# BolinLai/CSTS

Measured on AMD Instinct MI355X. Metric: clips/sec training (fwd+bwd) CSTS-Ego4D 16x256^2 bf16, higher is better.
Workload: dtype bf16; 1 GPU; CSTS_Ego4D_Gaze_Forecast.yaml train step (fwd + KLDiv + 0.05*EgoNCE + bwd + clip + AdamW), 16x256^2 video + 24 kHz STFT audio, b=4/GPU; mode=train, global_batch=4, frames=16, crop=256, parallelism=dp1, step=hip_graph, hip_graph=True, rccl_ranks=1

## Files before the change

csts_amd/csrc/attention.hip:

```cpp
#include <type_traits>
#include <utility>
#include "common.h"

#ifndef CSTS_ATTN_PART
#define CSTS_ATTN_PART 0
#endif
#ifndef CSTS_DKV_DEPTH
#define CSTS_DKV_DEPTH 4
#endif
#ifndef CSTS_DKV_SWZ
#define CSTS_DKV_SWZ 0
#endif

#ifdef CSTS_ATTN_STAMPS
#if CSTS_ATTN_PART == 1
__device__ unsigned long long g_attn_stamps[4096];
#else
static __device__ unsigned long long g_attn_stamps[4096];
#endif
#define AT_STAMP() do { if (stamp_on && nstamp < 4000) g_attn_stamps[nstamp++] = (unsigned long long)__builtin_amdgcn_s_memtime(); } while (0)
#if CSTS_ATTN_PART == 1
extern "C" int csts_debug_attn_stamps(unsigned long long* dst_host) {
  return (int)hipMemcpyFromSymbol(dst_host, HIP_SYMBOL(g_attn_stamps), sizeof(unsigned long long) * 4096);
}
// ... 1430 lines not shown
  CSTS_REQUIRE(strides_ok((a)->q_strides, (a)->dtype) && strides_ok((a)->k_strides, (a)->dtype) &&      \
                   strides_ok((a)->v_strides, (a)->dtype),                                             \
               "strides must keep 16-byte row alignment");                                              \
  if ((a)->mask_mode == CSTS_MASK_SPATIAL)                                                              \
  CSTS_REQUIRE((a)->mask_HW > 0 && (a)->Nq < (1 << 20) && (a)->Nq == (a)->mask_T * (a)->mask_HW + (a)->mask_T && (a)->Nk == (a)->Nq, "spatial mask needs Nq == Nk == T*HW + T < 2^20")

template <int HD, bool F32>
static bool launch_fwd(const AttnRoute& r, const AttnP& p, dim3 grid, hipStream_t stream) {
  const size_t sm = smem_fwd<HD, F32>();
  if (r.fwd == FWD_FAST) hipLaunchKernelGGL(attn_fwd_fast_kernel, grid, dim3(256), sm, stream, p);
  else hipLaunchKernelGGL((attn_fwd_kernel<HD, F32>), grid, dim3(256), sm, stream, p);
  return true;
}
template <int HD, bool F32>
static bool launch_dq(const AttnRoute& r, const AttnP& p, dim3 grid, hipStream_t stream) {
  const size_t sm = smem_bwd<HD, F32>();
  if (r.dq == DQ_FAST128) {
    constexpr size_t sm4 = (size_t)2 * 128 * 2 * Cfg<96, false>::LD_ROW * 2;
    if (!csts_dyn_lds_optin(reinterpret_cast<const void*>(&attn_dq_fast_kernel<4>), (int)sm4)) return false;
    hipLaunchKernelGGL(attn_dq_fast_kernel<4>, grid, dim3(256), sm4, stream, p);
  } else if (r.dq == DQ_FAST64) hipLaunchKernelGGL(attn_dq_fast_kernel<2>, grid, dim3(256), sm, stream, p);
  else hipLaunchKernelGGL((attn_dq_kernel<HD, F32>), grid, dim3(256), sm, stream, p);
  return true;
}
template <int HD, bool F32>
static bool launch_dkv(const AttnRoute& r, const AttnP& p, dim3 grid, hipStream_t stream) {
  const size_t sm = smem_bwd<HD, F32>() + (size_t)Cfg<HD, F32>::KVBLK * 4 * sizeof(float);
  if (r.dkv == DKV_FAST) return csts_attn_dkv_fast_launch(p, grid, stream);
  if constexpr (HD == 192 && !F32) {
    if (r.dkv == DKV_PLAIN) {
      hipLaunchKernelGGL((attn_dkv_kernel<192, false, false>), grid, dim3(256), sm, stream, p);
      return true;
    }
  }
  hipLaunchKernelGGL((attn_dkv_kernel<HD, F32, true>), grid, dim3(256), sm, stream, p);
  return true;
}
#define LAUNCH_BY_TYPE(fn, a, ...)                                                                                   \
  ((a)->head_dim == 96 ? ((a)->dtype == CSTS_F32 ? fn<96, true>(__VA_ARGS__) : fn<96, false>(__VA_ARGS__))           \
                       : ((a)->dtype == CSTS_F32 ? fn<192, true>(__VA_ARGS__) : fn<192, false>(__VA_ARGS__)))

static void launch_reduce(const csts_attn_args* a, const AttnP& p, hipStream_t stream) {
  const int64_t total = (int64_t)2 * a->B * a->H * a->Nk * a->head_dim / 8;
  hipLaunchKernelGGL(attn_dkv_reduce_kernel, dim3((unsigned)std::min<int64_t>(cdiv(total, 256), 4096)), dim3(256), 0, stream, p,
                     a->head_dim);
}

extern "C" int csts_attn_fwd(const csts_attn_args* a, hipStream_t stream) {
  ATTN_COMMON_CHECKS(a);
  CSTS_REQUIRE(a->O && a->LSE && aligned16(a->O) && strides_ok(a->o_strides, a->dtype), "bad output");
  AttnP p; fill(a, p);
  AttnRoute r;
  CSTS_REQUIRE(attn_route(a, &r), "no route");
  dim3 grid((unsigned)cdiv(a->Nq, 128), a->H, a->B);
  CSTS_REQUIRE(LAUNCH_BY_TYPE(launch_fwd, a, r, p, grid, stream), "hipFuncSetAttribute(MaxDynamicSharedMemorySize) failed on this device");
  CSTS_LAUNCH_CHECK();
  return 0;
}

extern "C" size_t csts_attn_bwd_workspace(const csts_attn_args* a) {
  AttnRoute r;
  return attn_route(a, &r) ? r.ws_bytes : 0;
}

extern "C" int csts_attn_route(const csts_attn_args* a, char* buf, int buflen, int* nsplit, int* q_chunk) {
  CSTS_REQUIRE(buf != nullptr && buflen > 0 && nsplit != nullptr && q_chunk != nullptr, "null pointer");
  AttnRoute r;
  CSTS_REQUIRE(attn_route(a, &r), "no route: null args, empty problem, or head_dim not 96 / 192");
  *nsplit = r.nsplit;
  *q_chunk = r.q_chunk;
  const int hd = a->head_dim;
  const char* t = a->dtype == CSTS_BF16 ? "false" : "true";
  char fwd[48] = "attn_fwd_fast_kernel", dq[48] = "", dkv[48] = "attn_bwd_fused_kernel";
  if (r.fwd == FWD_GENERIC) snprintf(fwd, sizeof fwd, "attn_fwd_kernel<%d,%s>", hd, t);
  if (r.dq == DQ_GENERIC) snprintf(dq, sizeof dq, "attn_dq_kernel<%d,%s>", hd, t);
  else if (r.dq != DQ_NONE) snprintf(dq, sizeof dq, "attn_dq_fast_kernel<%d>", r.dq == DQ_FAST128 ? 4 : 2);
  if (r.dkv == DKV_SLOW) snprintf(dkv, sizeof dkv, "attn_dkv_kernel<%d,%s,true>", hd, t);
  else if (r.dkv != DKV_ONE_PASS) snprintf(dkv, sizeof dkv, "attn_dkv_kernel<%d,false,false>", hd);
  const int n = snprintf(buf, buflen, "%s;%s;%s;%s", fwd, dq, dkv, r.nsplit > 1 ? "attn_dkv_reduce_kernel" : "");
  CSTS_REQUIRE(n < buflen, "buffer too small");
  return 0;
}

extern "C" int csts_attn_bwd(const csts_attn_args* a, void* workspace, size_t ws_bytes, hipStream_t stream) {
  ATTN_COMMON_CHECKS(a);
  CSTS_REQUIRE(a->O && a->LSE && a->dO && a->delta && a->dQ && a->dK && a->dV, "null backward operand");
  CSTS_REQUIRE(aligned16(a->dO) && aligned16(a->dQ) && aligned16(a->dK) && aligned16(a->dV), "alignment");
  CSTS_REQUIRE(strides_ok(a->do_strides, a->dtype) && strides_ok(a->dq_strides, a->dtype) &&
                   strides_ok(a->dk_strides, a->dtype) && strides_ok(a->dv_strides, a->dtype) &&
                   strides_ok(a->o_strides, a->dtype), "strides must keep 16-byte row alignment");
  AttnP p; fill(a, p);
  AttnRoute r;
  CSTS_REQUIRE(attn_route(a, &r), "no route");
  p.nsplit = r.nsplit; p.q_chunk = r.q_chunk;
  if (r.nsplit > 1) {
    if (workspace == nullptr || ws_bytes < r.ws_bytes) CSTS_FAIL("workspace too small [workspace != nullptr && ws_bytes >= csts_attn_bwd_workspace(a)]");
    p.ws = reinterpret_cast<float*>(workspace);
  }
  if (r.dkv == DKV_ONE_PASS) {
    hipLaunchKernelGGL((attn_bwd_fused_kernel<96>), dim3((unsigned)p.nsplit, (unsigned)(a->B * a->H)), dim3(256), 0, stream, p);
  } else {
    dim3 grid_dq((unsigned)cdiv(a->Nq, 128), a->H, a->B);
    CSTS_REQUIRE(LAUNCH_BY_TYPE(launch_dq, a, r, p, grid_dq, stream), "hipFuncSetAttribute(MaxDynamicSharedMemorySize) failed on this device");
    CSTS_LAUNCH_CHECK();
    dim3 grid_dkv((unsigned)cdiv(a->Nk, 128), p.nsplit, a->B * a->H);
    CSTS_REQUIRE(LAUNCH_BY_TYPE(launch_dkv, a, r, p, grid_dkv, stream), "hipFuncSetAttribute(MaxDynamicSharedMemorySize) failed on this device");
  }
  CSTS_LAUNCH_CHECK();
  if (r.nsplit > 1) {
    launch_reduce(a, p, stream);
    CSTS_LAUNCH_CHECK();
  }
  return 0;
}

extern "C" int csts_attn_probs(const csts_attn_args* a, float* probs, hipStream_t stream) {
  ATTN_COMMON_CHECKS(a);
  CSTS_REQUIRE(a->LSE && probs, "null pointer");
  AttnP p; fill(a, p);
  const int64_t total = (int64_t)a->B * a->H * a->Nq * a->Nk;
  hipLaunchKernelGGL(attn_probs_kernel, dim3((unsigned)std::min<int64_t>(cdiv(total, 256), 4096)), dim3(256), 0, stream, p,
                     a->head_dim, probs);
  CSTS_LAUNCH_CHECK();
  return 0;
}
#else
}
bool csts_attn_dkv_fast_launch(const csts_attn::AttnP& p, dim3 grid, hipStream_t stream) {
  constexpr size_t smf = (size_t)2 * 128 * 2 * (CSTS_DKV_SWZ ? 128 : Cfg<96, false>::LD_ROW) * 2 + 2 * 2 * 128 * sizeof(float);
  if (!csts_dyn_lds_optin(reinterpret_cast<const void*>(&attn_dkv_kernel<96, false, false>), (int)smf)) return false;
  hipLaunchKernelGGL((attn_dkv_kernel<96, false, false>), grid, dim3(256), smf, stream, p);
  return true;
}
#endif
```

csts_amd/csrc/norm.hip:

```cpp
#include "common.h"

#include <utility>

namespace {

constexpr int MAXV = 12;
constexpr int LN_BWD_WAVES = 8;

template <bool F32> __device__ __forceinline__ float ldt(const void* p, int64_t i) {
  if constexpr (F32) return reinterpret_cast<const float*>(p)[i];
  else return h16_lo((unsigned)reinterpret_cast<const unsigned short*>(p)[i]);
}
template <bool F32> __device__ __forceinline__ void stt(void* p, int64_t i, float v) {
  if constexpr (F32) reinterpret_cast<float*>(p)[i] = v;
  else reinterpret_cast<bf16*>(p)[i] = (bf16)v;
}
template <bool F32> __device__ __forceinline__ void ld8t(const void* p, int64_t i, float (&o)[8]) {
  if constexpr (F32) {
    const float4* q = reinterpret_cast<const float4*>(reinterpret_cast<const float*>(p) + i);
    const float4 a = q[0], b = q[1];
    o[0] = a.x; o[1] = a.y; o[2] = a.z; o[3] = a.w; o[4] = b.x; o[5] = b.y; o[6] = b.z; o[7] = b.w;
  } else {
    const uint4 r = *reinterpret_cast<const uint4*>(reinterpret_cast<const bf16*>(p) + i);
    o[0] = h16_lo(r.x); o[1] = h16_hi(r.x);
    o[2] = h16_lo(r.y); o[3] = h16_hi(r.y);
    o[4] = h16_lo(r.z); o[5] = h16_hi(r.z);
    o[6] = h16_lo(r.w); o[7] = h16_hi(r.w);
  }
}
template <bool F32> __device__ __forceinline__ void st8t(void* p, int64_t i, const float (&o)[8]) {
  if constexpr (F32) {
    float4* q = reinterpret_cast<float4*>(reinterpret_cast<float*>(p) + i);
    q[0] = make_float4(o[0], o[1], o[2], o[3]);
    q[1] = make_float4(o[4], o[5], o[6], o[7]);
  } else {
    bf16x8 v;
#pragma unroll
    for (int j = 0; j < 8; ++j) v[j] = (bf16)o[j];
    *reinterpret_cast<bf16x8*>(reinterpret_cast<bf16*>(p) + i) = v;
  }
}
template <int W, bool F32> __device__ __forceinline__ void ldw(const void* p, int64_t i, float (&o)[W]) {
  if constexpr (W == 8) ld8t<F32>(p, i, o);
  else o[0] = ldt<F32>(p, i);
}
template <int W, bool F32> __device__ __forceinline__ void stw(void* p, int64_t i, const float (&o)[W]) {
  if constexpr (W == 8) st8t<F32>(p, i, o);
  else stt<F32>(p, i, o[0]);
}
template <int GL> __device__ __forceinline__ float group_sum(float v) {
#pragma unroll
  for (int o = GL / 2; o > 0; o >>= 1) v += __shfl_xor(v, o, 64);
  return v;
}

__device__ __forceinline__ int64_t xcd_block(int64_t bid, int64_t nwg) {
#ifdef CSTS_LN_NO_XCD_MAP
  return bid;
#else
  const int64_t q = nwg >> 3, r = nwg & 7, xcd = bid & 7, slot = bid >> 3;
  return (xcd < r ? xcd * (q + 1) : r * (q + 1) + (xcd - r) * q) + slot;
#endif
}

template <int W, int GL, int NCH> struct Lane {
  int sub, C;
  int c0[W == 8 ? NCH : 1];
  bool act[W == 8 ? NCH : 1];
  __device__ __forceinline__ void form(int i) {
    if constexpr (W == 8) {
      const int c = (sub + GL * i) * 8;
      act[i] = c < C;
      c0[i] = min(c, C - 8);
    }
  }
  __device__ __forceinline__ bool on(int i) const {
    if constexpr (W == 8) return act[i];
    else return sub + GL * i < C;
  }
  __device__ __forceinline__ int st(int i) const {
    if constexpr (W == 8) return c0[i];
    else return sub + GL * i;
  }
  __device__ __forceinline__ int at(int i) const {
    if constexpr (W == 8) return c0[i];
    else return min(sub + GL * i, C - 1);
  }
  __device__ __forceinline__ void param(const float* p, int i, float (&o)[W]) const {
    if constexpr (W == 8) ld8t<true>(p, at(i), o);
    else o[0] = on(i) ? p[sub + GL * i] : 0.f;
  }
};

struct FwdAdd {
  const void* addend = nullptr;
  void* sum = nullptr;
};
template <int W, int GL, int NCH, int R, bool XF32, bool YF32>
__global__ __launch_bounds__(256) void ln_fwd_kernel(const void* __restrict__ x, const float* __restrict__ gamma,
                                                     const float* __restrict__ beta, void* __restrict__ y,
                                                     float* __restrict__ mean, float* __restrict__ rstd, int64_t rows,
                                                     int C, float eps, FwdAdd fa) {
  const int64_t bid = W == 8 ? xcd_block(blockIdx.x, gridDim.x) : (int64_t)blockIdx.x;
  const int64_t grp = (bid * 256 + threadIdx.x) / GL, ngrp = (int64_t)gridDim.x * 256 / GL;
  Lane<W, GL, NCH> ln{(int)(threadIdx.x % GL), C};
  float gm[NCH][W], bt[NCH][W];
#pragma unroll
  for (int i = 0; i < NCH; ++i) {
    ln.form(i);
    ln.param(gamma, i, gm[i]);
    ln.param(beta, i, bt[i]);
  }
  const float invC = 1.f / C;
  for (int64_t row0 = grp * R; row0 < rows; row0 += ngrp * R) {
    float v[R][NCH][W];
#pragma unroll
    for (int r = 0; r < R; ++r) {
      const int64_t row = min(row0 + r, rows - 1);
#pragma unroll
      for (int i = 0; i < NCH; ++i) {
        ldw<W, XF32>(x, row * C + ln.at(i), v[r][i]);
        if (fa.addend) {
          float a2[W];
          ldw<W, XF32>(fa.addend, row * C + ln.at(i), a2);
#pragma unroll
          for (int j = 0; j < W; ++j) {
            v[r][i][j] += a2[j];
            if constexpr (!XF32) v[r][i][j] = (float)(bf16)v[r][i][j];
          }
          if (ln.on(i) && row0 + r < rows) stw<W, XF32>(fa.sum, row * C + ln.st(i), v[r][i]);
        }
      }
    }
    constexpr int PH = W == 8 ? 1 : 3;
    float mu[R], rs[R];
#pragma unroll
    for (int ph = 0; ph < PH; ++ph)
#pragma unroll
      for (int r = 0; r < R; ++r) {
        if (PH == 1 || ph == 0) {
          float s = 0.f;
#pragma unroll
          for (int i = 0; i < NCH; ++i)
            if (ln.on(i)) {
#pragma unroll
              for (int j = 0; j < W; ++j) s += v[r][i][j];
            }
          mu[r] = group_sum<GL>(s) * invC;
        }
        if (PH == 1 || ph == 1) {
          float q = 0.f;
#pragma unroll
          for (int i = 0; i < NCH; ++i)
            if (ln.on(i)) {
#pragma unroll
              for (int j = 0; j < W; ++j) { const float d = v[r][i][j] - mu[r]; q += d * d; }
            }
          rs[r] = rsqrtf(group_sum<GL>(q) * invC + eps);
        }
        const int64_t row = row0 + r;
        if ((PH == 1 || ph == 2) && row < rows) {
#pragma unroll
          for (int i = 0; i < NCH; ++i)
            if (ln.on(i)) {
              float o[W];
#pragma unroll
              for (int j = 0; j < W; ++j) o[j] = (v[r][i][j] - mu[r]) * rs[r] * gm[i][j] + bt[i][j];
              stw<W, YF32>(y, row * C + ln.st(i), o);
            }
          if (ln.sub == 0) {
            if (mean) mean[row] = mu[r];
            if (rstd) rstd[row] = rs[r];
          }
        }
      }
  }
}

struct Copy16 {
  bf16* p = nullptr;
  const float* scale = nullptr;
  int64_t rps = 1;
  const void* dy2 = nullptr;
};
#ifndef CSTS_LN_BWD_R
#define CSTS_LN_BWD_R 1
#endif
#ifndef CSTS_LN_BWD_MINW
#define CSTS_LN_BWD_MINW 1
#endif
template <int W, int GL, int NCH, int R, bool DYF32, bool XF32>
__global__ __launch_bounds__(512, CSTS_LN_BWD_MINW) void ln_bwd_kernel(const void* __restrict__ dy, const void* __restrict__ x,
                                                         const float* __restrict__ gamma, const float* __restrict__ mean,
                                                         const float* __restrict__ rstd, void* __restrict__ dx,
                                                         const void* __restrict__ addend, float* __restrict__ ws, int64_t rows,
                                                         int C, const float* __restrict__ gamma1, Copy16 dx16) {
  extern __shared__ __attribute__((aligned(16))) float red[];
  const int64_t ro = (int64_t)blockIdx.y * rows;
  if (blockIdx.y == 1) gamma = gamma1;
  ws += (int64_t)blockIdx.y * gridDim.x * 2 * C;
  const int gib = threadIdx.x / GL;
  constexpr int GPB = 512 / GL;
  const int64_t bid = W == 8 ? xcd_block(blockIdx.x, gridDim.x) : (int64_t)blockIdx.x;
  const int64_t grp = bid * GPB + gib, ngrp = (int64_t)gridDim.x * GPB;
  Lane<W, GL, NCH> ln{(int)(threadIdx.x % GL), C};
  float gm[NCH][W], dg[NCH][W], db[NCH][W];
#pragma unroll
  for (int i = 0; i < NCH; ++i) {
    ln.form(i);
    ln.param(gamma, i, gm[i]);
#pragma unroll
    for (int j = 0; j < W; ++j) { dg[i][j] = 0.f; db[i][j] = 0.f; }
  }
  const float invC = 1.f / C;
  for (int64_t row0 = grp * R; row0 < rows; row0 += ngrp * R) {
    float d[R][NCH][W], xv[R][NCH][W], ad[R][NCH][W], mu[R], rs[R];
#pragma unroll
    for (int r = 0; r < R; ++r) {
      const int64_t row = ro + min(row0 + r, rows - 1);
      mu[r] = mean[row];
      rs[r] = rstd[row];
#pragma unroll
      for (int i = 0; i < NCH; ++i) {
        ldw<W, DYF32>(dy, row * C + ln.at(i), d[r][i]);
        if (dx16.dy2) {
          float d2[W];
          ldw<W, DYF32>(dx16.dy2, row * C + ln.at(i), d2);
#pragma unroll
          for (int j = 0; j < W; ++j) d[r][i][j] += d2[j];
        }
        ldw<W, XF32>(x, row * C + ln.at(i), xv[r][i]);
        if (addend) ldw<W, XF32>(addend, row * C + ln.at(i), ad[r][i]);
        else {
#pragma unroll
          for (int j = 0; j < W; ++j) ad[r][i][j] = 0.f;
        }
      }
    }
#pragma unroll
    for (int r = 0; r < R; ++r) {
      const bool live = row0 + r < rows;
      float s1 = 0.f, s2 = 0.f;
      float xh[NCH][W], g[NCH][W];
#pragma unroll
      for (int i = 0; i < NCH; ++i) {
        const bool ok = live && ln.on(i);
#pragma unroll
        for (int j = 0; j < W; ++j) {
          const float dd = ok ? d[r][i][j] : 0.f;
          xh[i][j] = ok ? (xv[r][i][j] - mu[r]) * rs[r] : 0.f;
          g[i][j] = dd * gm[i][j];
          dg[i][j] += dd * xh[i][j];
          db[i][j] += dd;
          s1 += g[i][j];
          s2 += g[i][j] * xh[i][j];
        }
      }
      s1 = group_sum<GL>(s1) * invC;
      s2 = group_sum<GL>(s2) * invC;
      if (live) {
        const int64_t row = ro + row0 + r;
#pragma unroll
        for (int i = 0; i < NCH; ++i)
          if (ln.on(i)) {
            float o[W];
#pragma unroll
            for (int j = 0; j < W; ++j) o[j] = rs[r] * (g[i][j] - s1 - xh[i][j] * s2) + ad[r][i][j];
            stw<W, XF32>(dx, row * C + ln.st(i), o);
            if (dx16.p) {
              if (dx16.scale) {
                const float sc = dx16.scale[(row0 + r) / dx16.rps];
#pragma unroll
                for (int j = 0; j < W; ++j) o[j] *= sc;
              }
              stw<W, false>(dx16.p, row * C + ln.st(i), o);
            }
          }
      }
    }
  }
#pragma unroll
  for (int i = 0; i < NCH; ++i)
    if (ln.on(i)) {
#pragma unroll
      for (int j = 0; j < W; ++j) {
        red[gib * 2 * C + ln.st(i) + j] = dg[i][j];
        red[gib * 2 * C + C + ln.st(i) + j] = db[i][j];
      }
    }
  __syncthreads();
  for (int i = threadIdx.x; i < 2 * C; i += blockDim.x) {
    float t = 0.f;
#pragma unroll(W == 8 ? 4 : GPB)
    for (int k = 0; k < GPB; ++k) t += red[k * 2 * C + i];
    ws[(int64_t)blockIdx.x * 2 * C + i] = t;
  }
}

template <int RL>
__global__ void reduce_rows_kernel(const float* __restrict__ ws, float* __restrict__ out, int64_t nrows, int64_t ncols,
                                   float scale) {
  __shared__ float red[RL][33];
  const int tx = threadIdx.x & 31, ty = threadIdx.x >> 5;
  const int64_t j = (int64_t)blockIdx.x * 32 + tx;
  float s = 0.f;
  if (j < ncols) {
    int64_t i = ty;
    for (; i + 3 * RL < nrows; i += 4 * RL) {
      const float a = ws[i * ncols + j], b = ws[(i + RL) * ncols + j], c = ws[(i + 2 * RL) * ncols + j],
                  d = ws[(i + 3 * RL) * ncols + j];
      s += a; s += b; s += c; s += d;
    }
    for (; i < nrows; i += RL) s += ws[i * ncols + j];
  }
  red[ty][tx] = s;
  __syncthreads();
  if (ty == 0 && j < ncols) {
    float t = 0.f;
#pragma unroll
    for (int r = 0; r < RL; ++r) t += red[r][tx];
    out[j] = t * scale;
  }
}

__global__ __launch_bounds__(1024) void reduce_rows_batched_kernel(const csts_reduce_desc* __restrict__ descs) {
  __shared__ float red[32][33];
  const csts_reduce_desc d = descs[blockIdx.y];
  const int tx = threadIdx.x & 31, ty = threadIdx.x >> 5;
  const int64_t j = (int64_t)blockIdx.x * 32 + tx;
  if ((int64_t)blockIdx.x * 32 >= d.ncols) return;
  float s = 0.f;
  if (j < d.ncols) {
    int64_t i = ty;
    for (; i + 3 * 32 < d.nrows; i += 4 * 32) {
      const float a = d.ws[i * d.ncols + j], b = d.ws[(i + 32) * d.ncols + j], c = d.ws[(i + 64) * d.ncols + j],
                  e = d.ws[(i + 96) * d.ncols + j];
      s += a; s += b; s += c; s += e;
    }
    for (; i < d.nrows; i += 32) s += d.ws[i * d.ncols + j];
  }
  red[ty][tx] = s;
  __syncthreads();
  if (ty == 0 && j < d.ncols) {
    float t = 0.f;
#pragma unroll
    for (int r = 0; r < 32; ++r) t += red[r][tx];
    d.out[j] = t * d.scale;
  }
}

__global__ __launch_bounds__(256) void reduce_rows_wide_kernel(const csts_reduce_desc* __restrict__ descs) {
  const csts_reduce_desc d = descs[blockIdx.y];
  const int64_t nvec = d.ncols >> 2;
  for (int64_t v = (int64_t)blockIdx.x * 256 + threadIdx.x; v < nvec; v += (int64_t)gridDim.x * 256) {
    float4 s = make_float4(0.f, 0.f, 0.f, 0.f);
    const float4* p = reinterpret_cast<const float4*>(d.ws) + v;
    int64_t i = 0;
    for (; i + 3 < d.nrows; i += 4) {
      const float4 a = p[i * nvec], b = p[(i + 1) * nvec], c = p[(i + 2) * nvec], e = p[(i + 3) * nvec];
      s.x += a.x; s.y += a.y; s.z += a.z; s.w += a.w;
      s.x += b.x; s.y += b.y; s.z += b.z; s.w += b.w;
      s.x += c.x; s.y += c.y; s.z += c.z; s.w += c.w;
      s.x += e.x; s.y += e.y; s.z += e.z; s.w += e.w;
    }
    for (; i < d.nrows; ++i) {
      const float4 a = p[i * nvec];
      s.x += a.x; s.y += a.y; s.z += a.z; s.w += a.w;
    }
    reinterpret_cast<float4*>(d.out)[v] = make_float4(s.x * d.scale, s.y * d.scale, s.z * d.scale, s.w * d.scale);
  }
}

}

extern "C" int csts_reduce_rows_wide(const csts_reduce_desc* device_descs, int n, int64_t max_ncols, hipStream_t stream) {
  CSTS_REQUIRE(device_descs != nullptr && n > 0 && n < 65536 && max_ncols > 0, "bad args");
  const unsigned gx = (unsigned)std::min<int64_t>(cdiv(max_ncols / 4, 256), 4096);
  hipLaunchKernelGGL(reduce_rows_wide_kernel, dim3(gx, (unsigned)n), dim3(256), 0, stream, device_descs);
  CSTS_LAUNCH_CHECK();
  return 0;
}

extern "C" int csts_reduce_rows_batched(const csts_reduce_desc* device_descs, int n, int64_t max_ncols, hipStream_t stream) {
  CSTS_REQUIRE(device_descs != nullptr && n > 0 && n < 65536 && max_ncols > 0, "bad args");
  hipLaunchKernelGGL(reduce_rows_batched_kernel, dim3((unsigned)cdiv(max_ncols, 32), (unsigned)n), dim3(1024), 0, stream,
                     device_descs);
  CSTS_LAUNCH_CHECK();
  return 0;
}

int csts_reduce_rows_launch(const float* ws, float* out, int64_t nrows, int64_t ncols, float scale, hipStream_t s) {
  const dim3 grid((unsigned)cdiv(ncols, 32));
  if (nrows > 64) hipLaunchKernelGGL(reduce_rows_kernel<32>, grid, dim3(1024), 0, s, ws, out, nrows, ncols, scale);
  else if (nrows > 8) hipLaunchKernelGGL(reduce_rows_kernel<8>, grid, dim3(256), 0, s, ws, out, nrows, ncols, scale);
  else hipLaunchKernelGGL(reduce_rows_kernel<2>, grid, dim3(64), 0, s, ws, out, nrows, ncols, scale);
  return 0;
}

extern "C" int csts_reduce_rows(const float* ws, float* out, int64_t nrows, int64_t ncols, float scale,
                                hipStream_t stream) {
  CSTS_REQUIRE(ws && out && nrows > 0 && ncols > 0, "bad args");
  csts_reduce_rows_launch(ws, out, nrows, ncols, scale, stream);
  CSTS_LAUNCH_CHECK();
  return 0;
}

#ifndef CSTS_LN_FWD_R
#define CSTS_LN_FWD_R 2
#endif
#ifndef CSTS_LN_BWD_CAP
#define CSTS_LN_BWD_CAP 512
#endif
struct LnForm { int W, GL, NCH, R; };
template <bool BWD> static constexpr LnForm LN_FORMS[8] = {
    {8, 16, 1, BWD ? CSTS_LN_BWD_R : CSTS_LN_FWD_R}, {8, 32, 1, BWD ? CSTS_LN_BWD_R : CSTS_LN_FWD_R},
    {8, 64, 1, BWD ? CSTS_LN_BWD_R : CSTS_LN_FWD_R}, {8, 64, 2, BWD ? 1 : 2},
    {1, 64, 2, 4}, {1, 64, 3, 4}, {1, 64, 6, 2}, {1, 64, 12, 1}};
static size_t ln_bwd_lds(const LnForm& f, int C) { return (size_t)(512 / f.GL) * 2 * C * sizeof(float); }
static int ln_form(bool bwd, int C, bool aligned) {
  const int vec = C <= 128 ? 0 : (C <= 256 ? 1 : (C <= 512 ? 2 : 3));
  if (aligned && C % 8 == 0 && !(bwd && ln_bwd_lds(LN_FORMS<true>[vec], C) > 65536)) return vec;
  return 4 + (C <= 128 ? 0 : (C <= 192 ? 1 : (C <= 384 ? 2 : 3)));
}
static bool all_aligned16(std::initializer_list<const void*> ptrs) {
  for (const void* q : ptrs)
    if (q != nullptr && !aligned16(q)) return false;
  return true;
}
static int64_t ln_bwd_blocks(int64_t rows, int C) {
  return std::min<int64_t>(cdiv(rows, LN_BWD_WAVES * LN_FORMS<true>[ln_form(true, C, false)].R), CSTS_LN_BWD_CAP);
}
template <class F, int... K> static void ln_pick(int k, F&& launch, std::integer_sequence<int, K...>) {
  ((k == K ? launch(std::integral_constant<int, K>{}) : void()), ...);
}

extern "C" int csts_layernorm_fwd(const void* x, int x_dt, const float* gamma, const float* beta, void* y, int y_dt,
                                  float* mean, float* rstd, int64_t rows, int C, float eps, hipStream_t stream) {
  return csts_layernorm_fwd_add(x, nullptr, nullptr, x_dt, gamma, beta, y, y_dt, mean, rstd, rows, C, eps, stream);
}

extern "C" int csts_layernorm_fwd_add(const void* x, const void* addend, void* sum_out, int x_dt, const float* gamma,
                                      const float* beta, void* y, int y_dt, float* mean, float* rstd, int64_t rows, int C,
                                      float eps, hipStream_t stream) {
  CSTS_REQUIRE(x && gamma && beta && y, "null pointer");
  CSTS_REQUIRE((addend == nullptr) == (sum_out == nullptr), "addend and sum_out: both or neither");
  CSTS_REQUIRE(rows > 0 && C > 0 && C <= 64 * MAXV, "C must be in (0, 768]");
  FwdAdd fa;
  fa.addend = addend; fa.sum = sum_out;
  const int form = ln_form(false, C, all_aligned16({x, y, gamma, beta, addend, sum_out}));
  const LnForm& f = LN_FORMS<false>[form];
  const dim3 grid((unsigned)std::min<int64_t>(cdiv(rows * f.GL, 256 * f.R), 4096));
  ln_pick(4 * form + 2 * (x_dt == CSTS_F32) + (y_dt == CSTS_F32), [&](auto k) {
    constexpr LnForm F = LN_FORMS<false>[decltype(k)::value / 4];
    hipLaunchKernelGGL((ln_fwd_kernel<F.W, F.GL, F.NCH, F.R, (decltype(k)::value & 2) != 0, (decltype(k)::value & 1) != 0>), grid,
                       dim3(256), 0, stream, x, gamma, beta, y, mean, rstd, rows, C, eps, fa);
  }, std::make_integer_sequence<int, 32>{});
  CSTS_LAUNCH_CHECK();
  return 0;
}

extern "C" size_t csts_layernorm_bwd_workspace(int64_t rows, int C) {
  return (size_t)ln_bwd_blocks(rows, C) * 2 * C * sizeof(float);
}

static void ln_bwd_launch(int segs, bool aligned, const void* dy, int dy_dt, const void* x, int x_dt, const float* const (&gamma)[2],
                          const float* mean, const float* rstd, void* dx, const void* addend, float* const (&dgb)[2], float* ws,
                          int64_t rows, int C, Copy16 c16, hipStream_t stream) {
  const int form = ln_form(true, C, aligned);
  const int64_t nb = ln_bwd_blocks(rows, C);
  const dim3 grid((unsigned)nb, (unsigned)segs);
  const size_t sh = ln_bwd_lds(LN_FORMS<true>[form], C);
  ln_pick(4 * form + 2 * (dy_dt == CSTS_F32) + (x_dt == CSTS_F32), [&](auto k) {
    constexpr LnForm F = LN_FORMS<true>[decltype(k)::value / 4];
    hipLaunchKernelGGL((ln_bwd_kernel<F.W, F.GL, F.NCH, F.R, (decltype(k)::value & 2) != 0, (decltype(k)::value & 1) != 0>), grid,
                       dim3(512), sh, stream, dy, x, gamma[0], mean, rstd, dx, addend, ws, rows, C, gamma[1], c16);
  }, std::make_integer_sequence<int, 32>{});
  for (int s = 0; s < segs && dgb[0] != nullptr; ++s) csts_reduce_rows_launch(ws + s * nb * 2 * C, dgb[s], nb, 2 * C, 1.f, stream);
}

extern "C" int csts_layernorm_bwd(const void* dy, int dy_dt, const void* x, int x_dt, const float* gamma,
                                  const float* mean, const float* rstd, void* dx, int dx_dt, const void* addend,
                                  void* dx_bf16, float* dgamma, float* dbeta, void* workspace, size_t ws_bytes,
                                  int64_t rows, int C, hipStream_t stream) {
  return csts_layernorm_bwd_ex(dy, nullptr, dy_dt, x, x_dt, gamma, mean, rstd, dx, dx_dt, addend, dx_bf16, nullptr, 1, dgamma,
                               dbeta, workspace, ws_bytes, rows, C, stream);
}

extern "C" int csts_layernorm_bwd_ex(const void* dy, const void* dy2, int dy_dt, const void* x, int x_dt, const float* gamma,
                                     const float* mean, const float* rstd, void* dx, int dx_dt, const void* addend,
                                     void* dx_bf16, const float* copy_row_scale, int64_t rows_per_scale,
                                     float* dgamma, float* dbeta, void* workspace, size_t ws_bytes, int64_t rows,
                                     int C, hipStream_t stream) {
  CSTS_REQUIRE(dy && x && gamma && mean && rstd && dx && workspace, "null pointer");
  CSTS_REQUIRE(copy_row_scale == nullptr || (dx_bf16 != nullptr && rows_per_scale > 0), "copy scale needs the bf16 copy and rows_per_scale > 0");
  Copy16 c16;
  c16.p = reinterpret_cast<bf16*>(dx_bf16); c16.scale = copy_row_scale; c16.rps = rows_per_scale > 0 ? rows_per_scale : 1;
  c16.dy2 = dy2;
  CSTS_REQUIRE(rows > 0 && C > 0 && C <= 64 * MAXV, "C must be in (0, 768]");
  CSTS_REQUIRE((dgamma == nullptr) == (dbeta == nullptr), "dgamma and dbeta: both or neither (neither = deferred second stage)");
  CSTS_REQUIRE(dgamma == nullptr || dbeta == dgamma + C, "dgamma/dbeta must be one contiguous [2*C] buffer");
  CSTS_REQUIRE(dx_dt == x_dt, "dx must have the dtype of x");
  const int64_t nb = ln_bwd_blocks(rows, C);
  CSTS_REQUIRE(ws_bytes >= (size_t)nb * 2 * C * sizeof(float), "workspace too small");
  ln_bwd_launch(1, all_aligned16({dy, dy2, x, dx, addend, dx_bf16, gamma}), dy, dy_dt, x, x_dt, {gamma, nullptr}, mean, rstd, dx,
                addend, {dgamma, nullptr}, reinterpret_cast<float*>(workspace), rows, C, c16, stream);
  CSTS_LAUNCH_CHECK();
  return 0;
}

extern "C" int csts_layernorm_bwd2(const void* dy, int dy_dt, const void* x, int x_dt, const float* gamma0,
                                   const float* gamma1, const float* mean, const float* rstd, void* dx, int dx_dt,
                                   float* dgb0, float* dgb1, void* workspace, size_t ws_bytes, int64_t rows, int C,
                                   hipStream_t stream) {
// ... 12 lines not shown
```

csts_amd/csrc/stencil.hip:

```cpp
#include "common.h"
#include <algorithm>
#include <cstdlib>
#include <cstring>
#include <initializer_list>
#include <vector>

namespace {

struct Geom {
  int B, C, HD;
  int Tf, Hf, Wf;
  int Tc, Hc, Wc;
  int st, sh, sw;
  int64_t f_bs, f_ts;
  int64_t c_bs, c_ts;
};

constexpr int VEC = 4;

__device__ __forceinline__ void ld4(const void* p, int dt, int64_t i, float (&o)[4]) {
  if (dt == CSTS_F32) {
    float4 a = *reinterpret_cast<const float4*>(reinterpret_cast<const float*>(p) + i);
    o[0] = a.x; o[1] = a.y; o[2] = a.z; o[3] = a.w;
  } else {
    bf16x4 a = *reinterpret_cast<const bf16x4*>(reinterpret_cast<const bf16*>(p) + i);
    o[0] = (float)a[0]; o[1] = (float)a[1]; o[2] = (float)a[2]; o[3] = (float)a[3];
  }
}
__device__ __forceinline__ void st4(void* p, int dt, int64_t i, const float (&o)[4]) {
  if (dt == CSTS_F32) {
    *reinterpret_cast<float4*>(reinterpret_cast<float*>(p) + i) = make_float4(o[0], o[1], o[2], o[3]);
  } else {
    bf16x4 a;
    a[0] = (bf16)o[0]; a[1] = (bf16)o[1]; a[2] = (bf16)o[2]; a[3] = (bf16)o[3];
    *reinterpret_cast<bf16x4*>(reinterpret_cast<bf16*>(p) + i) = a;
  }
}

struct FastDiv { unsigned m; int sh; int d; };
__device__ __forceinline__ int fdiv(int n, const FastDiv& f) { return (int)(((unsigned long long)(unsigned)n * f.m) >> f.sh); }
struct RowGeom {
  Geom g;
  int lt, lh, lw;
  FastDiv dNc, dHc, dWc;
  FastDiv dNf, dHf, dWf;
  FastDiv dN2, dH2, dW2;
  FastDiv dC4, dC8, dHD, dHeads;
};
__device__ __forceinline__ void decompf(int bt, const FastDiv& dN, const FastDiv& dH, const FastDiv& dW, int& b, int& t, int& h, int& w) {
  b = fdiv(bt, dN);
  int o = bt - b * dN.d;
  const int q = fdiv(o, dW);
  w = o - q * dW.d;
  t = fdiv(q, dH);
  h = q - t * dH.d;
}

__device__ __forceinline__ void decomp(int bt, int ntok, int H, int W, int& b, int& t, int& h, int& w) {
  b = bt / ntok;
  int o = bt - b * ntok;
  w = o % W; o /= W;
  h = o % H;
  t = o / H;
}

template <bool F32> __device__ __forceinline__ const void* bptr(const void* p, int64_t off) {
  if constexpr (F32) return reinterpret_cast<const float*>(p) + off;
  else return reinterpret_cast<const bf16*>(p) + off;
}
template <bool F32> __device__ __forceinline__ void* bptr(void* p, int64_t off) {
  if constexpr (F32) return reinterpret_cast<float*>(p) + off;
  else return reinterpret_cast<bf16*>(p) + off;
}

template <int V, bool F32> struct Raw { unsigned w[F32 ? V : V / 2]; };
template <int V, bool F32> __device__ __forceinline__ Raw<V, F32> raw_load(const void* base, int i) {
  Raw<V, F32> r;
  if constexpr (F32) {
    const uint4* q = reinterpret_cast<const uint4*>(reinterpret_cast<const float*>(base) + i);
#pragma unroll
    for (int k = 0; k < V / 4; ++k) { const uint4 a = q[k]; r.w[4 * k] = a.x; r.w[4 * k + 1] = a.y; r.w[4 * k + 2] = a.z; r.w[4 * k + 3] = a.w; }
  } else if constexpr (V == 8) {
    const uint4 a = *reinterpret_cast<const uint4*>(reinterpret_cast<const bf16*>(base) + i);
// ... 189 lines not shown
          float v[V];
          raw_cvt<V, F32>(raw[kh * 3 + kw], v);
          fmav<V>(acc, v, &wls[tap * (HD + WPAD)]);
        }
    };
    if constexpr (ALL27) {
      Raw<V, F32> r0[9], r1[9], r2[9];
      bool t0, t1, t2;
      slice_load(0, r0, t0); slice_load(1, r1, t1); slice_load(2, r2, t2);
      slice_mac(0, r0, t0); slice_mac(1, r1, t1); slice_mac(2, r2, t2);
    } else {
#pragma unroll 1
      for (int kt = 0; kt < 3; ++kt) {
        Raw<V, F32> raw[9];
        bool tvk;
        slice_load(kt, raw, tvk);
        slice_mac(kt, raw, tvk);
      }
    }
    if constexpr (!F32) {
#pragma unroll
      for (int j = 0; j < V; ++j) acc[j] = (float)(bf16)acc[j];
    }
    float s1 = 0.f;
    if (active) {
#pragma unroll
      for (int j = 0; j < V; ++j) s1 += acc[j];
    }
#pragma unroll
    for (int o = GL / 2; o > 0; o >>= 1) s1 += __shfl_xor(s1, o, 64);
    const float mu = s1 * invHD;
    float s2 = 0.f;
    if (active) {
#pragma unroll
      for (int j = 0; j < V; ++j) { const float d = acc[j] - mu; s2 += d * d; }
    }
#pragma unroll
    for (int o = GL / 2; o > 0; o >>= 1) s2 += __shfl_xor(s2, o, 64);
    const float rs = rsqrtf(s2 * invHD + eps);
    if (active) {
      const int64_t off = (int64_t)b * g.c_bs + (int64_t)(bt - b * ntok) * cts + c;
      raw_store<V, F32>(sl.conv[slot], off, acc);
      const float* gp = sl.gamma[slot] + cl;
      const float* bp = sl.beta[slot] + cl;
      float y[V];
#pragma unroll
      for (int q = 0; q < V / 4; ++q) {
        const float4 gq = *reinterpret_cast<const float4*>(gp + 4 * q), bq = *reinterpret_cast<const float4*>(bp + 4 * q);
        y[4 * q + 0] = (acc[4 * q + 0] - mu) * rs * gq.x + bq.x; y[4 * q + 1] = (acc[4 * q + 1] - mu) * rs * gq.y + bq.y;
        y[4 * q + 2] = (acc[4 * q + 2] - mu) * rs * gq.z + bq.z; y[4 * q + 3] = (acc[4 * q + 3] - mu) * rs * gq.w + bq.w;
      }
      raw_store<V, F32>(sl.y[slot], off, y);
      if (lane_in == 0) {
        const int64_t row = (int64_t)bt * H + head;
        sl.mean[slot][row] = mu;
        sl.rstd[slot][row] = rs;
      }
    }
  }
}

template <int N>
__device__ __forceinline__ void axis_cand(int f, int s, int ls, int nc, int (&k)[N], int (&o)[N], bool (&ok)[N]) {
#pragma unroll
  for (int i = 0; i < N; ++i) {
    int kk, n;
    if (N == 3) { kk = i; n = f + 1 - i; }
    else if (N == 2) { kk = ((f + 1) & 1) + 2 * i; n = f + 1 - kk; }
    else if (ls >= 0) { kk = (f + 1) & (s - 1); n = f + 1 - kk; }
    else { kk = (f + 1) % s; n = f + 1 - kk; }
    const int oo = ls >= 0 ? (n >> ls) : (n >= 0 ? n / s : -1);
    ok[i] = kk <= 2 && n >= 0 && oo < nc;
    k[i] = min(kk, 2);
    o[i] = min(max(oo, 0), nc - 1);
  }
}

struct Slots2 {
  const void* src[2];
  void* dst[2];
  const float* w[2];
};

template <int NT, int NH, int NW, bool CF32, bool FF32, int V>
__global__ __launch_bounds__(256, CSTS_DW_WAVES) void dwconv_transposed_kernel(RowGeom rg, Slots2 sl) {
  extern __shared__ __attribute__((aligned(16))) float wl[];
  const void* __restrict__ coarse = sl.src[blockIdx.y];
  const float* __restrict__ w = sl.w[blockIdx.y];
  void* __restrict__ fine = sl.dst[blockIdx.y];
  const Geom& g = rg.g;
  stage_weights_z(w, wl, g.HD);
  const int CQ = g.C / V;
  const int ntok = g.Tf * g.Hf * g.Wf;
  const int total = g.B * ntok * CQ;
  const int fts = (int)g.f_ts, cts = (int)g.c_ts;
  for (int idx = blockIdx.x * blockDim.x + threadIdx.x; idx < total; idx += gridDim.x * blockDim.x) {
    const int bt = fdiv(idx, V == 8 ? rg.dC8 : rg.dC4);
    const int c = (idx - bt * CQ) * V, cw = c - fdiv(c, rg.dHD) * g.HD;
    int b, ft, fh, fw;
    decompf(bt, rg.dNf, rg.dHf, rg.dWf, b, ft, fh, fw);
    int kt[NT], ot[NT], kh[NH], oh[NH], kw[NW], ow[NW];
    bool vt[NT], vh[NH], vw[NW];
    axis_cand<NT>(ft, g.st, rg.lt, g.Tc, kt, ot, vt);
    axis_cand<NH>(fh, g.sh, rg.lh, g.Hc, kh, oh, vh);
    axis_cand<NW>(fw, g.sw, rg.lw, g.Wc, kw, ow, vw);
#pragma unroll
    for (int i = 0; i < NT; ++i) ot[i] *= g.Hc * g.Wc * cts;
#pragma unroll
    for (int i = 0; i < NH; ++i) oh[i] *= g.Wc * cts;
#pragma unroll
    for (int i = 0; i < NW; ++i) ow[i] = ow[i] * cts + c;
    const void* cb = bptr<CF32>(coarse, (int64_t)b * g.c_bs);
    float acc[V];
#pragma unroll
    for (int j = 0; j < V; ++j) acc[j] = 0.f;
#pragma unroll
    for (int a = 0; a < NT; ++a) {
      Raw<V, CF32> raw[NH * NW];
#pragma unroll
      for (int e = 0; e < NH; ++e)
#pragma unroll
        for (int f = 0; f < NW; ++f) raw[e * NW + f] = raw_load<V, CF32>(cb, ot[a] + oh[e] + ow[f]);
#pragma unroll
      for (int e = 0; e < NH; ++e)
#pragma unroll
        for (int f = 0; f < NW; ++f) {
          const int tap = (vt[a] && vh[e] && vw[f]) ? kt[a] * 9 + kh[e] * 3 + kw[f] : 27;
          float v[V];
          raw_cvt<V, CF32>(raw[e * NW + f], v);
          fmav<V>(acc, v, &wl[tap * (g.HD + WPAD) + cw]);
        }
    }
    raw_store<V, FF32>(bptr<FF32>(fine, (int64_t)b * g.f_bs), (bt - b * ntok) * fts + c, acc);
  }
}

template <int NT>
__global__ __launch_bounds__(256, CSTS_DW_WAVES) void dwconv_transposed_s22_kernel(RowGeom rg, Slots2 sl) {
  extern __shared__ __attribute__((aligned(16))) float wl[];
  const bf16* __restrict__ coarse = reinterpret_cast<const bf16*>(sl.src[blockIdx.y]);
  bf16* __restrict__ fine = reinterpret_cast<bf16*>(sl.dst[blockIdx.y]);
  const Geom& g = rg.g;
  stage_weights_z(sl.w[blockIdx.y], wl, g.HD);
  const int CQ = g.C / 8;
  const int H2 = g.Hf >> 1, W2 = g.Wf >> 1;
  const int nblk = g.Tf * H2 * W2;
  const int total = g.B * nblk * CQ;
  const int fts = (int)g.f_ts, cts = (int)g.c_ts;
  for (int idx = blockIdx.x * blockDim.x + threadIdx.x; idx < total; idx += gridDim.x * blockDim.x) {
    const int bt = fdiv(idx, rg.dC8);
    const int c = (idx - bt * CQ) * 8, cw = c - fdiv(c, rg.dHD) * g.HD;
    int b, ft, mh, mw;
    decompf(bt, rg.dN2, rg.dH2, rg.dW2, b, ft, mh, mw);
    int kt[NT], ot[NT];
    bool vt[NT];
    axis_cand<NT>(ft, g.st, rg.lt, g.Tc, kt, ot, vt);
    const bool vh1 = mh + 1 < g.Hc, vw1 = mw + 1 < g.Wc;
    const int oh0 = mh * g.Wc * cts, oh1 = min(mh + 1, g.Hc - 1) * g.Wc * cts;
    const int ow0 = mw * cts + c, ow1 = min(mw + 1, g.Wc - 1) * cts + c;
    const bf16* cb = coarse + (int64_t)b * g.c_bs;
    float o00[8], o01[8], o10[8], o11[8];
#pragma unroll
    for (int j = 0; j < 8; ++j) { o00[j] = 0.f; o01[j] = 0.f; o10[j] = 0.f; o11[j] = 0.f; }
    Raw<8, false> raw[NT][4];
#pragma unroll
    for (int a = 0; a < NT; ++a) {
      const int tb = ot[a] * g.Hc * g.Wc * cts;
      raw[a][0] = raw_load<8, false>(cb, tb + oh0 + ow0);
      raw[a][1] = raw_load<8, false>(cb, tb + oh0 + ow1);
      raw[a][2] = raw_load<8, false>(cb, tb + oh1 + ow0);
      raw[a][3] = raw_load<8, false>(cb, tb + oh1 + ow1);
    }
#pragma unroll
    for (int a = 0; a < NT; ++a) {
      float i00[8], i01[8], i10[8], i11[8];
      raw_cvt<8, false>(raw[a][0], i00);
      raw_cvt<8, false>(raw[a][1], i01);
      raw_cvt<8, false>(raw[a][2], i10);
      raw_cvt<8, false>(raw[a][3], i11);
      const int t9 = kt[a] * 9;
      auto wrow = [&](bool ok, int kh, int kw) { return &wl[(ok ? t9 + kh * 3 + kw : 27) * (g.HD + WPAD) + cw]; };
      const bool v = vt[a];
      fmav<8>(o00, i00, wrow(v, 1, 1));
      fmav<8>(o01, i00, wrow(v, 1, 2));
      fmav<8>(o01, i01, wrow(v && vw1, 1, 0));
      fmav<8>(o10, i00, wrow(v, 2, 1));
      fmav<8>(o10, i10, wrow(v && vh1, 0, 1));
      fmav<8>(o11, i00, wrow(v, 2, 2));
      fmav<8>(o11, i01, wrow(v && vw1, 2, 0));
      fmav<8>(o11, i10, wrow(v && vh1, 0, 2));
      fmav<8>(o11, i11, wrow(v && vh1 && vw1, 0, 0));
    }
    bf16* fb = fine + (int64_t)b * g.f_bs;
    const int f00 = ((ft * g.Hf + 2 * mh) * g.Wf + 2 * mw) * fts + c;
    raw_store<8, false>(fb, f00, o00);
    raw_store<8, false>(fb, f00 + fts, o01);
    raw_store<8, false>(fb, f00 + g.Wf * fts, o10);
    raw_store<8, false>(fb, f00 + g.Wf * fts + fts, o11);
  }
}

struct WgSlots2 {
  const void* fine[2];
  const void* coarse[2];
  float* ws[2];
};
template <bool FF32, bool CF32>
__device__ __forceinline__ void dwconv_wgrad_body(const Geom& g, const void* __restrict__ fine, const void* __restrict__ coarse,
                                                  float* __restrict__ ws, int slab, int chunk, int bx, int by, int nbx, int tx, int ty,
                                                  int lanes, int nthr, float* __restrict__ red) {
  const int cl = 2 * tx;
  const int c = bx * slab + cl;
  const int ntok = g.Tc * g.Hc * g.Wc;
  const int total = g.B * ntok;
  const int beg = by * chunk, end = ty < lanes ? min(total, beg + chunk) : 0;
  const int fts = (int)g.f_ts, cts = (int)g.c_ts;
  float a0[27], a1[27];
#pragma unroll
  for (int k = 0; k < 27; ++k) { a0[k] = 0.f; a1[k] = 0.f; }
  int b = 0, ot = 0, oh = 0, ow = 0;
  if (beg + ty < end) decomp(beg + ty, ntok, g.Hc, g.Wc, b, ot, oh, ow);
  const int tstep = lanes;
  const char* fbase = reinterpret_cast<const char*>(fine);
  const char* cbase = reinterpret_cast<const char*>(coarse);
  constexpr unsigned FES = FF32 ? 4u : 2u, CES = CF32 ? 4u : 2u;
  for (int bt = beg + ty; bt < end; bt += tstep) {
    unsigned tof[3], hx[9];
    bool tv[3], hxv[9];
    {
      unsigned hof[3], xof[3];
      bool hv[3], xv[3];
#pragma unroll
      for (int k = 0; k < 3; ++k) {
        const int t = ot * g.st - 1 + k, h = oh * g.sh - 1 + k, x = ow * g.sw - 1 + k;
        tv[k] = (unsigned)t < (unsigned)g.Tf; tof[k] = (unsigned)(min(max(t, 0), g.Tf - 1) * g.Hf * g.Wf * fts);
        hv[k] = (unsigned)h < (unsigned)g.Hf; hof[k] = (unsigned)(min(max(h, 0), g.Hf - 1) * g.Wf * fts);
        xv[k] = (unsigned)x < (unsigned)g.Wf; xof[k] = (unsigned)(min(max(x, 0), g.Wf - 1) * fts + c);
      }
      const unsigned boff = (unsigned)((int)g.f_bs * b);
#pragma unroll
      for (int kh = 0; kh < 3; ++kh)
#pragma unroll
        for (int kw = 0; kw < 3; ++kw) { hx[kh * 3 + kw] = boff + hof[kh] + xof[kw]; hxv[kh * 3 + kw] = hv[kh] && xv[kw]; }
    }
    float c0, c1;
    {
      const unsigned coff = ((unsigned)((int)g.c_bs * b) + (unsigned)((bt - b * ntok) * cts + c)) * CES;
      if constexpr (CF32) {
        const float2 v = *reinterpret_cast<const float2*>(cbase + coff);
        c0 = v.x; c1 = v.y;
      } else {
        const unsigned v = *reinterpret_cast<const unsigned*>(cbase + coff);
        c0 = h16_lo(v); c1 = h16_hi(v);
      }
    }
    if constexpr (FF32) {
      float2 raw[27];
#pragma unroll
      for (int kt = 0; kt < 3; ++kt)
#pragma unroll
        for (int j = 0; j < 9; ++j) raw[kt * 9 + j] = *reinterpret_cast<const float2*>(fbase + (tof[kt] + hx[j]) * FES);
#pragma unroll
      for (int kt = 0; kt < 3; ++kt)
#pragma unroll
        for (int j = 0; j < 9; ++j) {
          const int tap = kt * 9 + j;
          const bool ok = tv[kt] && hxv[j];
          a0[tap] += (ok ? raw[tap].x : 0.f) * c0;
          a1[tap] += (ok ? raw[tap].y : 0.f) * c1;
        }
    } else {
      unsigned raw[27];
#pragma unroll
      for (int kt = 0; kt < 3; ++kt)
#pragma unroll
        for (int j = 0; j < 9; ++j) raw[kt * 9 + j] = *reinterpret_cast<const unsigned*>(fbase + (tof[kt] + hx[j]) * FES);
#pragma unroll
      for (int kt = 0; kt < 3; ++kt)
#pragma unroll
        for (int j = 0; j < 9; ++j) {
          const int tap = kt * 9 + j;
// ... 430 lines not shown
  CSTS_REQUIRE((a)->fine_token_stride % 8 == 0 && (a)->coarse_token_stride % 8 == 0 &&                       \
                   (a)->fine_batch_stride % 8 == 0 && (a)->coarse_batch_stride % 8 == 0,                     \
               "strides must be multiples of 8 elements");                                                   \
  CSTS_REQUIRE((int64_t)(a)->Tf * (a)->Hf * (a)->Wf * (a)->fine_token_stride < ((int64_t)1 << 31) &&          \
                   (int64_t)(a)->Tc * (a)->Hc * (a)->Wc * (a)->coarse_token_stride < ((int64_t)1 << 31),      \
               "one batch element must span < 2^31 elements");                                               \
  CSTS_REQUIRE((int64_t)(a)->B * (a)->Tf * (a)->Hf * (a)->Wf * (a)->C < ((int64_t)1 << 31), "B*N*C must be < 2^31")

extern "C" int csts_dwconv_strided(const csts_dwconv_geom* a, const void* fine, int fine_dt, const float* weight,
                                   void* coarse, int coarse_dt, hipStream_t stream) {
  CHECK_GEOM(a);
  CSTS_REQUIRE(all_set({fine, weight, coarse}), "null pointer");
  CSTS_REQUIRE(aligned16({fine, coarse}), "tensors must be 16-byte aligned");
  RowGeom rg; fill_geom(a, rg);
  const bool ff = fine_dt == CSTS_F32, cf = coarse_dt == CSTS_F32;
  const int vec = (!ff && !cf) ? 8 : VEC;
  const int64_t total = (int64_t)a->B * a->Tc * a->Hc * a->Wc * (a->C / vec);
  const dim3 grid(grid_for_staged(total)), block(256);
  const size_t sm = staged_bytes(a->HD);
  if (ff && cf) hipLaunchKernelGGL((dwconv_strided_kernel<true, true, 4>), grid, block, sm, stream, rg, fine, weight, coarse);
  else if (!ff && !cf) hipLaunchKernelGGL((dwconv_strided_kernel<false, false, 8>), grid, block, sm, stream, rg, fine, weight, coarse);
  else if (ff) hipLaunchKernelGGL((dwconv_strided_kernel<true, false, 4>), grid, block, sm, stream, rg, fine, weight, coarse);
  else hipLaunchKernelGGL((dwconv_strided_kernel<false, true, 4>), grid, block, sm, stream, rg, fine, weight, coarse);
  CSTS_LAUNCH_CHECK();
  return 0;
}

static int transposed_launch(const csts_dwconv_geom* a, int nslots, const void* const* coarse, int coarse_dt,
                             const float* const* weight, void* const* fine, int fine_dt, hipStream_t stream) {
  CHECK_GEOM(a);
  CSTS_REQUIRE(nslots == 1 || nslots == 2, "nslots must be 1 or 2");
  Slots2 sl{};
  for (int i = 0; i < nslots; ++i) {
    CSTS_REQUIRE(all_set({fine[i], weight[i], coarse[i]}), "null pointer");
    CSTS_REQUIRE(aligned16({fine[i], coarse[i]}), "tensors must be 16-byte aligned");
    sl.src[i] = coarse[i]; sl.dst[i] = fine[i]; sl.w[i] = weight[i];
  }
  RowGeom rg; fill_geom(a, rg);
  CSTS_REQUIRE(coarse_dt == fine_dt, "transposed stencil: both tensors must have the same dtype");
  const bool f32 = fine_dt == CSTS_F32;
  const int64_t total = (int64_t)a->B * a->Tf * a->Hf * a->Wf * (a->C / (f32 ? VEC : 8));
  const dim3 grid(grid_for_staged(total), nslots), block(256);
  const size_t sm = staged_bytes(a->HD);
  auto nc = [](int st) { return st == 1 ? 3 : (st == 2 ? 2 : 1); };
  if (!f32 && a->sh == 2 && a->sw == 2 && a->Hf % 2 == 0 && a->Wf % 2 == 0) {
    const int64_t items = (int64_t)a->B * a->Tf * (a->Hf / 2) * (a->Wf / 2) * (a->C / 8);
    const dim3 grid2(grid_for_staged(items), nslots);
    if (nc(a->st) == 3) hipLaunchKernelGGL((dwconv_transposed_s22_kernel<3>), grid2, block, sm, stream, rg, sl);
    else if (nc(a->st) == 2) hipLaunchKernelGGL((dwconv_transposed_s22_kernel<2>), grid2, block, sm, stream, rg, sl);
    else hipLaunchKernelGGL((dwconv_transposed_s22_kernel<1>), grid2, block, sm, stream, rg, sl);
    CSTS_LAUNCH_CHECK();
    return 0;
  }
  const int key = nc(a->st) * 100 + nc(a->sh) * 10 + nc(a->sw);
#define TR_CASE(NT, NH, NW)                                                                                          \
  case NT * 100 + NH * 10 + NW:                                                                                      \
    if (f32) hipLaunchKernelGGL((dwconv_transposed_kernel<NT, NH, NW, true, true, 4>), grid, block, sm, stream, rg, sl); \
    else hipLaunchKernelGGL((dwconv_transposed_kernel<NT, NH, NW, false, false, 8>), grid, block, sm, stream, rg, sl);   \
    break;
  switch (key) {
    TR_CASE(3, 3, 3) TR_CASE(3, 3, 2) TR_CASE(3, 3, 1) TR_CASE(3, 2, 3) TR_CASE(3, 2, 2) TR_CASE(3, 2, 1)
    TR_CASE(3, 1, 3) TR_CASE(3, 1, 2) TR_CASE(3, 1, 1) TR_CASE(2, 3, 3) TR_CASE(2, 3, 2) TR_CASE(2, 3, 1)
    TR_CASE(2, 2, 3) TR_CASE(2, 2, 2) TR_CASE(2, 2, 1) TR_CASE(2, 1, 3) TR_CASE(2, 1, 2) TR_CASE(2, 1, 1)
    TR_CASE(1, 3, 3) TR_CASE(1, 3, 2) TR_CASE(1, 3, 1) TR_CASE(1, 2, 3) TR_CASE(1, 2, 2) TR_CASE(1, 2, 1)
    TR_CASE(1, 1, 3) TR_CASE(1, 1, 2) TR_CASE(1, 1, 1)
    default: CSTS_FAIL("unsupported stride combination");
  }
#undef TR_CASE
  CSTS_LAUNCH_CHECK();
  return 0;
}

extern "C" int csts_dwconv_transposed(const csts_dwconv_geom* a, const void* coarse, int coarse_dt, const float* weight,
                                      void* fine, int fine_dt, hipStream_t stream) {
  return transposed_launch(a, 1, &coarse, coarse_dt, &weight, &fine, fine_dt, stream);
}

extern "C" int csts_dwconv_transposed2(const csts_dwconv_geom* a, const void* const coarse[2], int coarse_dt,
                                       const float* const weight[2], void* const fine[2], int fine_dt, hipStream_t stream) {
  CSTS_REQUIRE(coarse && weight && fine, "null pointer");
  return transposed_launch(a, 2, coarse, coarse_dt, weight, fine, fine_dt, stream);
}

static void wgrad_plan(const csts_dwconv_geom* a, int& slab, int& nslab, int64_t& chunk, int64_t& nchunk) {
  int k = std::max(1, 192 / a->HD);
  while (k > 1 && a->C % (a->HD * k) != 0) --k;
  slab = a->HD * k;
  nslab = a->C / slab;
  const int64_t total = (int64_t)a->B * a->Tc * a->Hc * a->Wc;
  nchunk = std::max<int64_t>(1, std::min<int64_t>(512 / nslab, cdiv(total, 16)));
  chunk = cdiv(total, nchunk);
  nchunk = cdiv(total, chunk);
}

extern "C" size_t csts_dwconv_wgrad_workspace(const csts_dwconv_geom* a) {
  if (!a || a->C <= 0 || a->HD <= 0) return 0;
  int slab, nslab; int64_t chunk, nchunk;
  wgrad_plan(a, slab, nslab, chunk, nchunk);
  return (size_t)nchunk * nslab * a->HD * 27 * sizeof(float);
}

static int wgrad_launch(const csts_dwconv_geom* a, int nslots, const void* const* fine, int fine_dt, const void* const* coarse,
                        int coarse_dt, float* const* dweight, void* workspace, size_t ws_bytes, hipStream_t stream) {
  CHECK_GEOM(a);
  CSTS_REQUIRE(nslots == 1 || nslots == 2, "nslots must be 1 or 2");
  CSTS_REQUIRE(workspace != nullptr, "null workspace");
  int slab, nslab; int64_t chunk, nchunk;
  wgrad_plan(a, slab, nslab, chunk, nchunk);
  CSTS_REQUIRE(a->C % slab == 0 && slab % a->HD == 0 && slab % 2 == 0, "channel slab must hold whole heads");
  const size_t per_slot = (size_t)nchunk * nslab * a->HD * 27;
  CSTS_REQUIRE(ws_bytes >= per_slot * nslots * sizeof(float), "workspace too small");
  RowGeom rg; fill_geom(a, rg);
  WgSlots2 sl{};
  for (int i = 0; i < nslots; ++i) {
    CSTS_REQUIRE(all_set({fine[i], coarse[i]}), "null pointer");
    sl.fine[i] = fine[i]; sl.coarse[i] = coarse[i];
    sl.ws[i] = reinterpret_cast<float*>(workspace) + per_slot * i;
  }
  CSTS_REQUIRE(coarse_dt == fine_dt, "stencil wgrad: both tensors must have the same dtype");
  const int lanes = (int)std::max<int64_t>(1, std::min<int64_t>(std::min<int64_t>(8, 512 / (slab / 2)), chunk / 2));
  const dim3 wg(nslab, (unsigned)nchunk, nslots), wb(slab / 2, lanes);
  if (fine_dt == CSTS_F32) hipLaunchKernelGGL((dwconv_wgrad_kernel<true, true>), wg, wb, (size_t)slab * 27 * 4, stream, rg, sl, slab, (int)chunk);
  else hipLaunchKernelGGL((dwconv_wgrad_kernel<false, false>), wg, wb, (size_t)slab * 27 * 4, stream, rg, sl, slab, (int)chunk);
  CSTS_LAUNCH_CHECK();
  for (int i = 0; i < nslots; ++i) {
    if (dweight != nullptr && dweight[i] != nullptr) {
      csts_reduce_rows_launch(sl.ws[i], dweight[i], nchunk * nslab, (int64_t)a->HD * 27, 1.f, stream);
      CSTS_LAUNCH_CHECK();
    }
  }
  return 0;
}

extern "C" int csts_dwconv_wgrad(const csts_dwconv_geom* a, const void* fine, int fine_dt, const void* coarse,
                                 int coarse_dt, float* dweight, void* workspace, size_t ws_bytes, hipStream_t stream) {
  return wgrad_launch(a, 1, &fine, fine_dt, &coarse, coarse_dt, &dweight, workspace, ws_bytes, stream);
}

extern "C" int csts_dwconv_wgrad2(const csts_dwconv_geom* a, const void* const fine[2], int fine_dt, const void* const coarse[2],
                                  int coarse_dt, float* const dweight[2], void* workspace, size_t ws_bytes, hipStream_t stream) {
  CSTS_REQUIRE(fine && coarse, "null pointer");
  return wgrad_launch(a, 2, fine, fine_dt, coarse, coarse_dt, dweight, workspace, ws_bytes, stream);
}

static_assert(sizeof(WgItem) == CSTS_DWCONV_WGRAD_TABLE_ENTRY, "device table entry size is part of the C-ABI");

static int grouped_min_tokens() {
  static const int v = [] { const char* e = getenv("CSTS_SWG_TOKENS"); const int x = e ? atoi(e) : 0; return x >= 8 ? x : 64; }();
  return v;
}
static void wgrad_plan_grouped(const csts_dwconv_geom* a, int& slab, int& nslab, int64_t& chunk, int64_t& nchunk) {
  wgrad_plan(a, slab, nslab, chunk, nchunk);
  const int64_t total = (int64_t)a->B * a->Tc * a->Hc * a->Wc;
  nchunk = std::max<int64_t>(1, std::min<int64_t>(nchunk, cdiv(total, grouped_min_tokens())));
  chunk = cdiv(total, nchunk);
  nchunk = cdiv(total, chunk);
}
extern "C" size_t csts_dwconv_wgrad_grouped_workspace(const csts_dwconv_geom* a) {
  if (!a || a->C <= 0 || a->HD <= 0) return 0;
  int slab, nslab; int64_t chunk, nchunk;
  wgrad_plan_grouped(a, slab, nslab, chunk, nchunk);
  return (size_t)nchunk * nslab * a->HD * 27 * sizeof(float);
}

extern "C" int csts_dwconv_wgrad_grouped_plan(const csts_dwconv_wgrad_item* items, int nitems, void* table_host, size_t table_bytes,
                                              int* nblocks) {
// ... 155 lines not shown
```

csts_amd/lib.py:

```python
from __future__ import annotations

import ctypes as C
import os

_lib = None


class CstsError(RuntimeError):
    pass


_HERE = os.path.dirname(os.path.abspath(__file__))
LIB_PATH = os.environ.get("CSTS_HIP_LIB") or os.path.join(_HERE, "libcsts_hip.so")
HALF = os.environ.get("CSTS_HALF", "bf16")
_PATHS = {"bf16": LIB_PATH, "fp16": os.environ.get("CSTS_HIP_LIB_F16") or os.path.join(_HERE, "libcsts_hip_f16.so")}


def set_half(kind: str):
    global HALF, LIB_PATH
    if kind not in _PATHS:
        raise ValueError(f"16-bit type must be 'bf16' or 'fp16', got {kind!r}")
    if _lib is not None and kind != HALF:
        raise CstsError(f"this process already runs the {HALF} kernel library; the {kind} build is a different shared object "
                        "(one 16-bit activation type per process: start a new process for the other mode)")
# ... 82 lines not shown

class Im2colGeom(C.Structure):
    _fields_ = [("B", C.c_int), ("Cin", C.c_int), ("T", C.c_int), ("H", C.c_int), ("W", C.c_int),
                ("kernel", C.c_int * 3), ("stride", C.c_int * 3), ("padding", C.c_int * 3),
                ("To", C.c_int), ("Ho", C.c_int), ("Wo", C.c_int), ("Kpad", C.c_int)]


class TokenSegment(C.Structure):
    _fields_ = [("src", vp), ("dst", vp), ("src_bs", i64), ("dst_bs", i64), ("src_off", i64), ("dst_off", i64), ("n", C.c_int), ("pad_", C.c_int)]


class KvRowsGeom(C.Structure):
    _fields_ = [("B", C.c_int), ("C", C.c_int), ("T", C.c_int), ("H", C.c_int), ("W", C.c_int), ("sh", C.c_int), ("sw", C.c_int),
                ("Hc", C.c_int), ("Wc", C.c_int)]


class WgradItem(C.Structure):
    _fields_ = [("A", vp), ("B", vp), ("C", vp), ("colsum", vp), ("lda", i64), ("ldb", i64), ("ldc", i64),
                ("kbeg", i64), ("kend", i64), ("M", C.c_int), ("N", C.c_int), ("m0", C.c_int), ("n0", C.c_int)]


class ReduceDesc(C.Structure):
    _fields_ = [("ws", vp), ("out", vp), ("nrows", i64), ("ncols", i64), ("scale", C.c_float), ("pad_", C.c_int)]


class OptTensor(C.Structure):
    _fields_ = [("p", vp), ("m", vp), ("v", vp), ("w16", vp), ("n", i64), ("weight_decay", C.c_float), ("pad_", C.c_int)]


class OptArgs(C.Structure):
    _fields_ = [("chunk_tensor", vp), ("chunk_off", vp), ("nchunks", C.c_int), ("chunk_elems", C.c_int),
                ("tensors", vp), ("grads", vp), ("ntensors", C.c_int),
                ("partial", vp), ("state", vp), ("lr", vp),
                ("beta1", C.c_float), ("beta2", C.c_float), ("eps", C.c_float), ("max_grad_norm", C.c_float),
                ("grad_dt", C.c_int), ("scaler", vp), ("growth", C.c_float), ("backoff", C.c_float), ("growth_interval", C.c_int),
                ("extra_sq", vp), ("n_extra_sq", C.c_int)]


class OptFactored(C.Structure):
    _fields_ = [("p", vp), ("m", vp), ("v", vp), ("w16", vp), ("dy", vp), ("a", vp), ("a_dt", C.c_int),
                ("N", C.c_int), ("K", C.c_int), ("T", C.c_int), ("weight_decay", C.c_float), ("tensor", C.c_int)]


OPT_ADAMW, OPT_ADAM, OPT_SGD = 0, 1, 2


class OptRule(C.Structure):
    _fields_ = [("kind", C.c_int), ("momentum", C.c_float), ("dampening", C.c_float), ("nesterov", C.c_int),
                ("clip_value", C.c_float), ("pad_", C.c_int), ("buf_step", vp)]


_I, _F, _U32 = C.c_int, C.c_float, C.c_uint32
class TransposeTile(C.Structure):
    _fields_ = [("src", C.c_void_p), ("dst", C.c_void_p), ("R", C.c_int), ("C", C.c_int), ("r0", C.c_int), ("c0", C.c_int)]


SYMBOLS = {
    "csts_last_error": (C.c_char_p, []),
    "csts_abi_version": (_I, []),
    "csts_half_kind": (_I, []),
    "csts_gemm": (_I, [C.POINTER(GemmArgs), vp]),
    "csts_gemm_splitk_workspace": (sz, [i64, i64, i64, _I]),
    "csts_gemm_v2_eligible": (_I, [C.POINTER(GemmArgs)]),
    "csts_wgrad_grouped": (_I, [vp, _I, _I, _I, vp]),
    "csts_wgrad_grouped8": (_I, [vp, _I, vp]),
    "csts_wgrad_grouped8_limited": (_I, [vp, _I, _I, vp]),
    "csts_wgrad_grouped5": (_I, [vp, _I, vp]),
    "csts_gemm_kernel_name": (_I, [C.POINTER(GemmArgs), C.c_char_p, _I, C.POINTER(_I)]),
    "csts_gemm_plan": (_I, [C.POINTER(GemmArgs), C.POINTER(_I), C.POINTER(_I), C.POINTER(_I)]),
    "csts_layernorm_fwd": (_I, [vp, _I, vp, vp, vp, _I, vp, vp, i64, _I, _F, vp]),
    "csts_layernorm_fwd_add": (_I, [vp, vp, vp, _I, vp, vp, vp, _I, vp, vp, i64, _I, _F, vp]),
    "csts_layernorm_bwd_workspace": (sz, [i64, _I]),
    "csts_layernorm_bwd": (_I, [vp, _I, vp, _I, vp, vp, vp, vp, _I, vp, vp, vp, vp, vp, sz, i64, _I, vp]),
    "csts_layernorm_bwd_ex": (_I, [vp, vp, _I, vp, _I, vp, vp, vp, vp, _I, vp, vp, vp, i64, vp, vp, vp, sz, i64, _I, vp]),
    "csts_reduce_rows_batched": (_I, [vp, _I, i64, vp]),
    "csts_reduce_rows_wide": (_I, [vp, _I, i64, vp]),
    "csts_layernorm_bwd2": (_I, [vp, _I, vp, _I, vp, vp, vp, vp, vp, _I, vp, vp, vp, sz, i64, _I, vp]),
    "csts_reduce_rows": (_I, [vp, vp, i64, i64, _F, vp]),
    "csts_dwconv_strided": (_I, [C.POINTER(DwconvGeom), vp, _I, vp, vp, _I, vp]),
    "csts_dwconv_transposed": (_I, [C.POINTER(DwconvGeom), vp, _I, vp, vp, _I, vp]),
    "csts_dwconv_wgrad_workspace": (sz, [C.POINTER(DwconvGeom)]),
    "csts_dwconv_wgrad": (_I, [C.POINTER(DwconvGeom), vp, _I, vp, _I, vp, vp, sz, vp]),
    "csts_dwconv_transposed2": (_I, [C.POINTER(DwconvGeom), vp * 2, _I, vp * 2, vp * 2, _I, vp]),
    "csts_dwconv_wgrad2": (_I, [C.POINTER(DwconvGeom), vp * 2, _I, vp * 2, _I, vp * 2, vp, sz, vp]),
    "csts_dwconv_wgrad_grouped_workspace": (sz, [C.POINTER(DwconvGeom)]),
    "csts_dwconv_wgrad_grouped_plan": (_I, [C.POINTER(DwconvWgradItem), _I, vp, sz, C.POINTER(C.c_int)]),
    "csts_dwconv_wgrad_grouped": (_I, [vp, _I, _I, _I, vp]),
    "csts_pool_ln_fwd": (_I, [C.POINTER(PoolLnArgs), vp]),
    "csts_maxpool_fwd": (_I, [C.POINTER(PoolGeom), vp, _I, vp, vp, vp]),
    "csts_maxpool_bwd": (_I, [C.POINTER(PoolGeom), vp, _I, vp, vp, vp]),
    "csts_trilinear_fwd": (_I, [C.POINTER(PoolGeom), vp, _I, vp, _I, vp, _I, vp]),
    "csts_trilinear_bwd": (_I, [C.POINTER(PoolGeom), vp, _I, vp, _I, vp]),
    "csts_attn_fwd": (_I, [C.POINTER(AttnArgs), vp]),
    "csts_attn_bwd_workspace": (sz, [C.POINTER(AttnArgs)]),
    "csts_attn_bwd": (_I, [C.POINTER(AttnArgs), vp, sz, vp]),
    "csts_attn_probs": (_I, [C.POINTER(AttnArgs), vp, vp]),
    "csts_attn_route": (_I, [C.POINTER(AttnArgs), C.c_char_p, _I, C.POINTER(_I), C.POINTER(_I)]),
    "csts_im2col": (_I, [C.POINTER(Im2colGeom), vp, _I, vp, _I, vp]),
    "csts_posembed_build": (_I, [vp, vp, vp, _I, _I, _I, vp]),
    "csts_transpose_batched": (_I, [vp, _I, vp, _I, i64, _I, _I, vp]),
    "csts_transpose_multi": (_I, [vp, _I, vp]),
    "csts_colsum_workspace": (sz, [i64, i64, i64]),
    "csts_colsum": (_I, [vp, _I, vp, vp, i64, i64, i64, vp, sz, vp]),
    "csts_axpby": (_I, [vp, _I, vp, _I, vp, _I, i64, _F, _F, vp]),
    "csts_rows_gather": (_I, [C.POINTER(KvRowsGeom), vp, _I, vp, vp]),
    "csts_copy_token_segments": (_I, [C.POINTER(TokenSegment), _I, _I, _I, _I, vp]),
    "csts_rows_scatter_add": (_I, [C.POINTER(KvRowsGeom), vp, _I, vp, _I, vp]),
    "csts_scale_rows": (_I, [vp, _I, vp, i64, vp, _I, i64, i64, vp]),
    "csts_dropout_fwd": (_I, [vp, vp, vp, i64, vp, _I, vp, _U32, _U32, _F, i64, i64, vp]),
    "csts_dropout_bwd": (_I, [vp, _I, vp, i64, vp, _I, vp, _U32, _U32, _F, i64, i64, vp]),
    "csts_dropout_mask": (_I, [vp, _U32, _U32, vp, i64, vp]),
    "csts_dropout_mask_host": (_I, [_U32, _U32, _U32, _U32, C.c_uint64, i64, vp]),
    "csts_add2": (_I, [vp, _I, vp, _I, vp, vp, i64, vp]),
    "csts_add2_scaled_copy": (_I, [vp, _I, vp, _I, vp, vp, vp, i64, i64, vp]),
    "csts_rowdot2": (_I, [vp, _I, vp, _I, vp, i64, _I, vp]),
    "csts_audio_attn_fwd": (_I, [vp, _I, vp, vp, _I, _I, _I, _I, _I, _F, vp]),
    "csts_audio_attn_bwd": (_I, [vp, _I, vp, vp, _I, _I, _I, _I, _I, _F, vp]),
    "csts_reweight_fwd": (_I, [vp, vp, vp, i64, _I, _I, vp]),
    "csts_reweight_bwd": (_I, [vp, vp, vp, vp, vp, i64, _I, _I, vp]),
    "csts_token_mean_fwd": (_I, [vp, vp, i64, _I, _I, vp]),
    "csts_token_mean_bwd": (_I, [vp, vp, i64, _I, _I, vp]),
    "csts_rowdot_fwd": (_I, [vp, _I, vp, vp, vp, i64, _I, vp]),
    "csts_rowdot_dx": (_I, [vp, vp, vp, _I, i64, _I, vp]),
    "csts_softmax_fwd": (_I, [vp, vp, i64, _I, _F, vp]),
    "csts_softmax_bwd": (_I, [vp, vp, vp, i64, _I, _F, vp]),
    "csts_kldiv_fwd": (_I, [vp, vp, vp, vp, i64, _I, _F, vp]),
    "csts_kldiv_bwd": (_I, [vp, vp, vp, vp, i64, _I, _F, vp]),
    "csts_rownorm_fwd": (_I, [vp, vp, vp, i64, _I, _F, vp]),
    "csts_rownorm_bwd": (_I, [vp, vp, vp, vp, i64, _I, _F, vp]),
    "csts_egonce_fwd": (_I, [vp, vp, vp, vp, _I, _F, vp]),
    "csts_egonce_bwd": (_I, [vp, vp, vp, vp, vp, _I, _F, vp]),
    "csts_adamw_step": (_I, [C.POINTER(OptArgs), vp]),
    "csts_factored_sqnorm_workspace": (sz, [C.POINTER(OptFactored), _I]),
    "csts_factored_sqnorm": (_I, [C.POINTER(OptFactored), _I, vp, vp, sz, vp]),
    "csts_adamw_factored": (_I, [C.POINTER(OptFactored), _I, vp, vp, _F, _F, _F, vp]),
    "csts_opt_step": (_I, [C.POINTER(OptArgs), C.POINTER(OptRule), vp]),
    "csts_opt_factored_step": (_I, [C.POINTER(OptFactored), _I, C.POINTER(OptRule), vp, vp, _F, _F, _F, vp]),
    "csts_frames_normalize": (_I, [vp, vp, _I, i64, _I, C.c_float * 3, C.c_float * 3, vp]),
    "csts_stft_frames": (_I, [_I, _I, _I]),
    "csts_stft_logpower": (_I, [vp, vp, _I, _I, _I, _I, _I, _F, vp]),
    "csts_audio_windows": (_I, [vp, vp, vp, _I, _I, _I, _I, _I, vp]),
    "csts_gaze_heatmaps": (_I, [vp, _I, vp, i64, _I, _I, _I, vp]),
    "csts_spatial_params": (_I, [vp, vp, _I, _I, _I, _I, _I, _I, _I, _I, _I, _I, _I, vp, vp, vp]),
    "csts_spatial_sample": (_I, [vp, vp, vp, _I, _I, _I, _I, _I, C.c_float * 3, C.c_float * 3, vp]),
    "csts_clip_sample": (_I, [vp, i64, vp, vp, vp, _I, _I, _I, _I, _I, C.c_float * 3, C.c_float * 3, vp]),
    "csts_spatial_rule_host": (_I, [vp, _I, _I, _I, _I, _I, _I, _I, _I, _I, _I, _I, vp, vp, vp]),
    "csts_spatial_uniforms_host": (_I, [_U32, _U32, C.c_uint64, i64, vp]),
    "csts_batch_params": (_I, [vp, vp, vp, _I, _I, _I, _I, _I, _I, _I, _I, _I, vp, vp, vp]),
    "csts_batch_sample": (_I, [vp, i64, vp, vp, vp, vp, _I, _I, _I, _I, C.c_float * 3, C.c_float * 3, vp]),
    "csts_audio_gather": (_I, [vp, vp, vp, vp, _I, _I, _I, _I, vp]),
    "csts_resample_len": (i64, [i64, _I, _I]),
    "csts_resample_wav": (_I, [vp, _I, _I, _I, i64, vp, _I, _I, _I, vp, vp]),
    "csts_resample_ready": (i64, [i64, _I, _I, _I, _I]),
    "csts_resample_first_input": (i64, [i64, _I, _I, _I]),
    "csts_resample_stream": (_I, [vp, _I, _I, i64, i64, i64, vp, _I, _I, _I, i64, i64, vp, vp]),
    "csts_yuv_to_rgb": (_I, [vp, vp, i64, _I, _I, _I, _I, _I, vp]),
    "csts_yuv_to_rgb_host": (_I, [vp, vp, i64, _I, _I, _I, _I, _I]),
    "csts_rgb_to_yuv": (_I, [vp, vp, i64, _I, _I, _I, _I, _I, vp]),
    "csts_rgb_to_yuv_host": (_I, [vp, vp, i64, _I, _I, _I, _I, _I]),
    "csts_spatial_sample_yuv": (_I, [vp, vp, vp, _I, _I, _I, _I, _I, C.c_float * 3, C.c_float * 3, _I, _I, _I, vp]),
    "csts_clip_sample_yuv": (_I, [vp, i64, vp, vp, vp, _I, _I, _I, _I, _I, C.c_float * 3, C.c_float * 3, _I, _I, _I, vp]),
    "csts_batch_sample_yuv": (_I, [vp, i64, vp, vp, vp, vp, _I, _I, _I, _I, C.c_float * 3, C.c_float * 3, _I, _I, _I, vp]),
    "csts_stream_stft": (_I, [vp, i64, i64, i64, i64, i64, vp, _I, _I, _I, _I, _F, vp]),
    "csts_stream_audio_windows": (_I, [vp, _I, i64, vp, vp, _I, _I, _I, _I, vp]),
    "csts_stream_ingest": (_I, [vp, _I, _I, _I, vp, _I, vp, vp, _I, _I, C.c_float * 3, C.c_float * 3, vp]),
    "csts_stream_ingest_yuv": (_I, [vp, _I, _I, _I, vp, _I, vp, vp, _I, _I, C.c_float * 3, C.c_float * 3, _I, _I, _I, vp]),
    "csts_stream_gather": (_I, [vp, _I, vp, vp, _I, _I, _I, vp]),
    "csts_group_stft": (_I, [vp, vp, _I, vp, _I, _I, _I, _I, _I, _F, vp]),
    "csts_group_audio_windows": (_I, [vp, _I, _I, vp, vp, vp, vp, _I, _I, _I, _I, vp]),
    "csts_group_ingest": (_I, [vp, vp, _I, vp, vp, _I, vp, i64, _I, C.c_float * 3, C.c_float * 3, vp]),
    "csts_group_ingest_yuv": (_I, [vp, vp, _I, vp, vp, _I, vp, i64, _I, C.c_float * 3, C.c_float * 3, _I, _I, _I, vp]),
    "csts_live_track_add": (_I, [vp, vp, _I, _I, _I, vp, vp, vp, _I, vp]),
    "csts_live_track_rows": (_I, [vp, vp, vp, _I, i64, _I, _I, _I, _I, _I, vp, vp, vp, vp, vp, vp, vp]),
    "csts_group_live_add": (_I, [vp, vp, vp, _I, _I, _I, vp, vp, vp, _I, _I, vp]),
    "csts_group_live_rows": (_I, [vp, vp, vp, _I, _I, vp, vp, _I, _I, _I, _I, _I, vp, vp, vp, vp, vp, vp, vp]),
    "csts_adaptive_f1_workspace": (sz, [i64, _I]),
    "csts_adaptive_f1": (_I, [vp, vp, vp, vp, _I, i64, _I, _I, vp, vp, sz, vp]),
    "csts_f1_counts": (_I, [vp, vp, vp, _I, i64, _I, _I, vp, vp]),
# ... 50 lines not shown
```

csts_amd/ops.py:

```python
from __future__ import annotations

import collections
import contextlib
import ctypes as C
import functools
import math
import os
import weakref
from typing import Optional, Sequence, Tuple

import torch
from torch.autograd import Function

from . import lib as L

F32, BF16 = L.F32, L.BF16


def _lib():
    return L.load()


def _dt(t: torch.Tensor) -> int:
    if t.dtype == torch.float32:
# ... 977 lines not shown
        M, K, Hd, N, rps, compute, has_res = ctx.meta
        sc = (row_scale, rps) if row_scale is not None else None
        drop = ctx.drop
        d16 = _grad16(dy, compute, sc) if (dy.is_contiguous() and drop is None) else None
        dy = dy.contiguous()
        if drop is not None:
            dys = _dropout_bwd(dy, drop.at(1), row_scale, rps, out_dt=BF16 if (compute == BF16 and BF16_GRAD_COPY) else None)
        elif d16 is not None:
            dys = d16
        elif row_scale is not None:
            dys = scale_rows(dy, row_scale, rps, M, N, out_dt=BF16 if (compute == BF16 and BF16_GRAD_COPY) else None)
        else:
            dys = dy
        P1, pb1, P2, pb2 = ctx.params
        dW2, db2 = _wgrad(dys, g, M, N, Hd, compute, want_bias=True, params=(P2, pb2))
        dh = torch.empty_like(h)
        _dgrad(dys, W2, ctx.w16t[1], dh, M, N, Hd, compute, epilogue=L.EPI_DGELU, aux=h)
        if drop is not None:
            _dropout_bwd(dh, drop, inplace=True)
        dW1, db1 = _wgrad(dh, x, M, Hd, K, compute, want_bias=True, params=(P1, pb1))
        dx = None
        if ctx.needs_input_grad[0]:
            dx = torch.empty_like(x)
            _dgrad(dh, W1, ctx.w16t[0], dx, M, Hd, K, compute)
        return dx, dW1, db1, dW2, db2, (dy if has_res else None), None, None, None, None, None, None, None, None, None, None


def mlp(x, W1, b1, W2, b2, *, residual=None, row_scale=None, rows_per_scale=1, act_dt=F32, out_dt=F32, compute=F32,
        w16_1=None, w16_2=None, w16t_1=None, w16t_2=None, drop: Optional[Dropout] = None):
    y = MlpFn.apply(x, W1, b1, W2, b2, residual, row_scale, rows_per_scale, act_dt, out_dt, compute, w16_1, w16_2,
                    w16t_1, w16t_2, drop)
    if drop is not None:
        return y
    return _mark_scaled_output(y, row_scale if residual is not None else None, rows_per_scale)


def _conv_geom(B, Cc, HD, fine_thw, stride, f_bs, f_ts, c_bs, c_ts) -> L.DwconvGeom:
    g = L.DwconvGeom()
    g.B, g.C, g.HD = B, Cc, HD
    g.Tf, g.Hf, g.Wf = fine_thw
    g.st, g.sh, g.sw = stride
    g.Tc, g.Hc, g.Wc = [(f - 1) // s + 1 for f, s in zip(fine_thw, stride)]
    g.fine_batch_stride, g.fine_token_stride = f_bs, f_ts
    g.coarse_batch_stride, g.coarse_token_stride = c_bs, c_ts
    return g


def _ln_rows_fwd(c, gamma, beta, HD, act_dt):
    rows = c.numel() // HD
    y = torch.empty(c.shape, dtype=torch_dtype(act_dt), device=c.device)
    mean = torch.empty(rows, dtype=torch.float32, device=c.device)
    rstd = torch.empty_like(mean)
    L.check(_lib().csts_layernorm_fwd(_p(c), _dt(c), _p(gamma), _p(beta), _p(y), act_dt, _p(mean), _p(rstd), rows, HD, 1e-5,
                                      _stream()), "csts_layernorm_fwd(head)")
    return y, mean, rstd


def _ln_rows_bwd(dy, c, gamma, mean, rstd, HD, params=None):
    rows = c.numel() // HD
    dc, dgb = _ln_bwd_call(dy, c, gamma, mean, rstd, None, rows, HD, "csts_layernorm_bwd(head)", params=params)
    if dgb is None:
        return dc, None, None
    return dc, dgb[:HD], dgb[HD:]


def _attn_args(dt, dims, mask, qd, kd, vd, o=None, lse=None, do=None, delta=None, tq=None, tk=None, tv=None):
    B, H, Nq, Nk, HD = dims
    a = L.AttnArgs()
    a.dtype, a.B, a.H, a.Nq, a.Nk, a.head_dim = dt, B, H, Nq, Nk, HD
    for name, d in (("Q", qd), ("K", kd), ("V", vd), ("dQ", tq), ("dK", tk), ("dV", tv)):
        if d is not None:
            setattr(a, name, _p(d[0], d[1]))
            setattr(a, name.lower() + "_strides", (C.c_int64 * 3)(*d[2]))
    a.O, a.LSE, a.dO, a.delta = _p(o), _p(lse), _p(do), _p(delta)
    if o is not None:
        a.o_strides = (C.c_int64 * 3)(Nq * H * HD, H * HD, HD)
    if do is not None:
        a.do_strides = (C.c_int64 * 3)(Nq * H * HD, H * HD, HD)
    a.scale = HD ** -0.5
    a.mask_mode, a.mask_T, a.mask_HW = mask
    return a


class AttnInnerFn(Function):

    @staticmethod
    def forward(ctx, qkv, kvc, wq, gq, bq, wk, gk, bk, wv, gv, bv, meta):
        _need_gpu(qkv)
        (B, N, Cc, H, thw, kind, stride_q, stride_kv, has_pool_q, has_pool_kv, mask_mode, mask_T, mask_HW, act_dt) = meta
        qkv = qkv.contiguous()
        HD = Cc // H
        dev = qkv.device
        lib = _lib()
        s = _stream()
        saved = {}
        QW = Cc if kvc is not None else 3 * Cc
        if kvc is not None:
            kvc = kvc.contiguous()
            kv_thw = [thw[0]] + list(kv_compact_dims(thw, stride_kv))
            assert has_pool_kv and kv_thw[0] * kv_thw[1] * kv_thw[2] == kvc.shape[1] and kvc.shape[2] == 2 * Cc
            kv_src, kv_off, kv_w, kv_n, kv_stride = kvc, (0, Cc), 2 * Cc, kvc.shape[1], (1, 3, 3)
        else:
            kv_thw, kv_src, kv_off, kv_w, kv_n, kv_stride = list(thw), qkv, (Cc, 2 * Cc), 3 * Cc, N, stride_kv

        def slot_view(slot):
            return (qkv, slot * Cc, (N * QW, QW, HD), N)

        def pooled(slot, w, gamma, beta, stride, transposed):
            if transposed:
                fine_thw = [t * st for t, st in zip(thw, stride)]
                Nf = fine_thw[0] * fine_thw[1] * fine_thw[2]
                g = _conv_geom(B, Cc, HD, fine_thw, stride, Nf * Cc, Cc, N * QW, QW)
                c = torch.empty(B, Nf, Cc, dtype=qkv.dtype, device=dev)
                L.check(lib.csts_dwconv_transposed(C.byref(g), _p(qkv, slot * Cc), _dt(qkv), _p(w), _p(c), _dt(c), s),
                        "csts_dwconv_transposed")
                n_out = Nf
                out_thw = fine_thw
            else:
                g = _conv_geom(B, Cc, HD, list(thw), stride, N * QW, QW, 0, Cc)
                n_out = g.Tc * g.Hc * g.Wc
                g.coarse_batch_stride = n_out * Cc
                c = torch.empty(B, n_out, Cc, dtype=qkv.dtype, device=dev)
                L.check(lib.csts_dwconv_strided(C.byref(g), _p(qkv, slot * Cc), _dt(qkv), _p(w), _p(c), _dt(c), s),
                        "csts_dwconv_strided")
                out_thw = [g.Tc, g.Hc, g.Wc]
            y, mean, rstd = _ln_rows_fwd(c, gamma, beta, HD, act_dt)
            saved[slot] = (c, mean, rstd, g)
            return (y, 0, (n_out * Cc, Cc, HD), n_out), out_thw

        def pooled_fused(slots, ws_, gammas, betas, stride):
            ns = len(slots)
            if slots[0] == 0:
                src, offs, g = qkv, (0,), _conv_geom(B, Cc, HD, list(thw), stride, N * QW, QW, 0, Cc)
            else:
                src, offs, g = kv_src, kv_off, _conv_geom(B, Cc, HD, kv_thw, kv_stride, kv_n * kv_w, kv_w, 0, Cc)
            n_out = g.Tc * g.Hc * g.Wc
            g.coarse_batch_stride = n_out * Cc
            rows = B * n_out * H
            c = torch.empty(ns, B, n_out, Cc, dtype=qkv.dtype, device=dev)
            y = torch.empty_like(c)
            mean = torch.empty(ns, rows, dtype=torch.float32, device=dev)
            rstd = torch.empty_like(mean)
            pa = L.PoolLnArgs()
            pa.geom, pa.nslots, pa.dt, pa.eps = g, ns, _dt(qkv), 1e-5
            for i, slot in enumerate(slots):
                pa.fine[i], pa.weight[i], pa.gamma[i], pa.beta[i] = _p(src, offs[i]), _p(ws_[i]), _p(gammas[i]), _p(betas[i])
                pa.conv_out[i], pa.y[i], pa.mean[i], pa.rstd[i] = _p(c[i]), _p(y[i]), _p(mean[i]), _p(rstd[i])
            L.check(lib.csts_pool_ln_fwd(C.byref(pa), s), "csts_pool_ln_fwd")
            for i, slot in enumerate(slots):
                saved[slot] = (c[i], mean[i], rstd[i], g)
            if ns == 2:
                saved["kv"] = (c, mean, rstd, g)
            return [(y[i], 0, (n_out * Cc, Cc, HD), n_out) for i in range(ns)]

        if kind == "dec":
            qd, _ = pooled(0, wq, gq, bq, stride_q, True)
        elif has_pool_q:
            qd, = pooled_fused([0], [wq], [gq], [bq], stride_q)
        else:
            qd = slot_view(0)
        if has_pool_kv:
            kd, vd = pooled_fused([1, 2], [wk, wv], [gk, gv], [bk, bv], stride_kv)
        else:
            kd, vd = slot_view(1), slot_view(2)
        Nq, Nk = qd[3], kd[3]
        o = torch.empty(B, Nq, Cc, dtype=qkv.dtype, device=dev)
        lse = torch.empty(B, H, Nq, dtype=torch.float32, device=dev)
        a = _attn_args(_dt(qkv), (B, H, Nq, Nk, HD), (mask_mode, mask_T, mask_HW), qd, kd, vd, o=o, lse=lse)
        L.check(lib.csts_attn_fwd(C.byref(a), s), "csts_attn_fwd")
        ctx.meta = meta
        ctx.saved_slots = saved
        ctx.descr = (qd, kd, vd, Nq, Nk)
        ctx.save_for_backward(qkv, o, lse, wq, gq, wk, gk, wv, gv, kvc)
        ctx.params = (wq, gq, bq, wk, gk, bk, wv, gv, bv)
        ctx.mark_non_differentiable(lse)
        ctx.set_materialize_grads(False)
        return o, lse

    @staticmethod
    def backward(ctx, do, _dlse):
        (B, N, Cc, H, thw, kind, stride_q, stride_kv, has_pool_q, has_pool_kv, mask_mode, mask_T, mask_HW, act_dt) = ctx.meta
        qkv, o, lse, wq, gq, wk, gk, wv, gv, kvc = ctx.saved_tensors
        qd, kd, vd, Nq, Nk = ctx.descr
        saved = ctx.saved_slots
        HD = Cc // H
        dev = qkv.device
        lib = _lib()
        s = _stream()
        do = do.contiguous()
        dqkv = torch.empty_like(qkv)
        QW = Cc if kvc is not None else 3 * Cc
        if kvc is not None:
            dkvc = torch.empty_like(kvc)
            kv_fine, kv_dfine, kv_off = kvc, dkvc, (0, Cc)
        else:
            dkvc, kv_fine, kv_dfine, kv_off = None, qkv, dqkv, (Cc, 2 * Cc)
        delta = torch.empty(B, H, Nq, dtype=torch.float32, device=dev)

        def grad_target(slot, n_rows):
            if slot in saved:
                t = torch.empty(B, n_rows, Cc, dtype=qkv.dtype, device=dev)
                return t, 0, (n_rows * Cc, Cc, HD)
            return dqkv, slot * Cc, (N * QW, QW, HD)

        tq = grad_target(0, Nq)
        if "kv" in saved:
            dkv = torch.empty(2, B, Nk, Cc, dtype=qkv.dtype, device=dev)
            tk, tv = (dkv[0], 0, (Nk * Cc, Cc, HD)), (dkv[1], 0, (Nk * Cc, Cc, HD))
        else:
            tk, tv = grad_target(1, Nk), grad_target(2, Nk)
        a = _attn_args(_dt(qkv), (B, H, Nq, Nk, HD), (mask_mode, mask_T, mask_HW), qd, kd, vd, o=o, lse=lse, do=do, delta=delta,
                       tq=tq, tk=tk, tv=tv)
        ws = _ws(lib.csts_attn_bwd_workspace(C.byref(a)), dev)
        L.check(lib.csts_attn_bwd(C.byref(a), _p(ws), ws.numel(), s), "csts_attn_bwd")

        grads = {}

        P = ctx.params

        def pooled_bwd(slot, dy, w, gamma, transposed):
            c, mean, rstd, g = saved[slot]
            pw, pg, pb = P[3 * slot], P[3 * slot + 1], P[3 * slot + 2]
            dc, dg, db = _ln_rows_bwd(dy, c, gamma, mean, rstd, HD, params=(pg, pb))
            defer = _can_defer(pw)
            grouped = defer and _stencil_group_now()
            wsz = (lib.csts_dwconv_wgrad_grouped_workspace if grouped else lib.csts_dwconv_wgrad_workspace)(C.byref(g))
            wws = _ws(wsz, dev)
            dw = torch.empty(HD * 27, dtype=torch.float32, device=dev)
            dwp = None if defer else _p(dw)
            if grouped:
                if transposed:
                    _queue_stencil_wgrad(g, dc, 0, qkv, slot * Cc, wws)
                else:
                    _queue_stencil_wgrad(g, qkv, slot * Cc, dc, 0, wws)
            elif transposed:
                L.check(lib.csts_dwconv_wgrad(C.byref(g), _p(dc), _dt(dc), _p(qkv, slot * Cc), _dt(qkv), dwp, _p(wws),
                                              wws.numel(), s), "csts_dwconv_wgrad")
            else:
                L.check(lib.csts_dwconv_wgrad(C.byref(g), _p(qkv, slot * Cc), _dt(qkv), _p(dc), _dt(dc), dwp, _p(wws),
                                              wws.numel(), s), "csts_dwconv_wgrad")
            if transposed:
                L.check(lib.csts_dwconv_strided(C.byref(g), _p(dc), _dt(dc), _p(w), _p(dqkv, slot * Cc), _dt(dqkv), s),
                        "csts_dwconv_strided(bwd)")
            else:
                L.check(lib.csts_dwconv_transposed(C.byref(g), _p(dc), _dt(dc), _p(w), _p(dqkv, slot * Cc), _dt(dqkv), s),
                        "csts_dwconv_transposed(bwd)")
            dwv = dw.view(HD, 1, 3, 3, 3)
            if defer:
                _defer(wws, dw, wsz // (HD * 27 * 4), HD * 27)
                _assign_later(pw, dwv)
                dwv = None
            grads[slot] = (dwv, dg, db)

        def pooled_bwd_kv():
            c2, mean2, rstd2, g = saved["kv"]
            rows = B * Nk * H
            dc2 = torch.empty_like(c2)
            dgb = torch.empty(2, 2 * HD, dtype=torch.float32, device=dev)
            nbytes = lib.csts_layernorm_bwd_workspace(rows, HD)
            lws = _ws(2 * nbytes, dev)
            defer = _can_defer(P[3], P[4], P[5], P[6], P[7], P[8])
            L.check(lib.csts_layernorm_bwd2(_p(dkv), _dt(dkv), _p(c2), _dt(c2), _p(gk), _p(gv), _p(mean2), _p(rstd2), _p(dc2),
                                            _dt(dc2), None if defer else _p(dgb[0]), None if defer else _p(dgb[1]), _p(lws),
                                            lws.numel(), rows, HD, s), "csts_layernorm_bwd2")
            if defer:
                nrow = nbytes // (2 * HD * 4)
                _defer(lws[:nbytes], dgb[0], nrow, 2 * HD)
                _defer(lws[nbytes:], dgb[1], nrow, 2 * HD)
            vp2 = C.c_void_p * 2
            L.check(lib.csts_dwconv_transposed2(C.byref(g), vp2(_p(dc2[0]), _p(dc2[1])), _dt(dc2), vp2(_p(wk), _p(wv)),
                                                vp2(_p(kv_dfine, kv_off[0]), _p(kv_dfine, kv_off[1])), _dt(kv_dfine), s),
                    "csts_dwconv_transposed2")
            grouped = defer and _stencil_group_now()
            wsz = (lib.csts_dwconv_wgrad_grouped_workspace if grouped else lib.csts_dwconv_wgrad_workspace)(C.byref(g))
            wws = _ws(2 * wsz, dev)
            dw = torch.empty(2, HD * 27, dtype=torch.float32, device=dev)
            dwp = vp2(None, None) if defer else vp2(_p(dw[0]), _p(dw[1]))
            if grouped:
                for i in (0, 1):
                    _queue_stencil_wgrad(g, kv_fine, kv_off[i], dc2[i], 0, wws[i * wsz:(i + 1) * wsz])
            else:
                L.check(lib.csts_dwconv_wgrad2(C.byref(g), vp2(_p(kv_fine, kv_off[0]), _p(kv_fine, kv_off[1])), _dt(kv_fine),
                                               vp2(_p(dc2[0]), _p(dc2[1])), _dt(dc2), dwp, _p(wws), wws.numel(), s), "csts_dwconv_wgrad2")
            if defer:
                nrow = wsz // (HD * 27 * 4)
                _defer(wws[:wsz], dw[0], nrow, HD * 27)
                _defer(wws[wsz:], dw[1], nrow, HD * 27)
            for i, slot in enumerate((1, 2)):
                gw, gg, gb = dw[i].view(HD, 1, 3, 3, 3), dgb[i, :HD], dgb[i, HD:]
                if defer:
                    _assign_later(P[3 * slot], gw)
                    _assign_later(P[3 * slot + 1], gg)
                    _assign_later(P[3 * slot + 2], gb)
                    gw = gg = gb = None
                grads[slot] = (gw, gg, gb)

        if 0 in saved:
            pooled_bwd(0, tq[0], wq, gq, kind == "dec")
        if "kv" in saved:
            pooled_bwd_kv()
        elif 1 in saved:
            pooled_bwd(1, tk[0], wk, gk, False)
            pooled_bwd(2, tv[0], wv, gv, False)
        gq_ = grads.get(0, (None, None, None))
        gk_ = grads.get(1, (None, None, None))
        gv_ = grads.get(2, (None, None, None))
        return (dqkv, dkvc, gq_[0], gq_[1], gq_[2], gk_[0], gk_[1], gk_[2], gv_[0], gv_[1], gv_[2], None)


def attention_inner(qkv, wq, gq, bq, wk, gk, bk, wv, gv, bv, meta, kvc=None):
    return AttnInnerFn.apply(qkv, kvc, wq, gq, bq, wk, gk, bk, wv, gv, bv, meta)


KV_COMPACT_MIN_STRIDE = int(os.environ.get("CSTS_KV_COMPACT", "8"))


def kv_compact_dims(thw, stride_kv):
    out = []
    for n, st in zip(thw[1:], stride_kv[1:]):
        no = (n - 1) // st + 1
        out.append(3 * no - 1 - (1 if (no - 1) * st + 1 > n - 1 else 0))
    return tuple(out)


def kv_compact_ok(thw, stride_kv, has_pool_kv) -> bool:
    return bool(has_pool_kv and KV_COMPACT_MIN_STRIDE > 0 and stride_kv[0] == 1 and stride_kv[1] >= max(3, KV_COMPACT_MIN_STRIDE)
                and stride_kv[2] >= max(3, KV_COMPACT_MIN_STRIDE))


def _kv_rows_geom(B, Cc, thw, stride_kv) -> L.KvRowsGeom:
    g = L.KvRowsGeom()
    g.B, g.C, g.T, g.H, g.W = B, Cc, thw[0], thw[1], thw[2]
    g.sh, g.sw = stride_kv[1], stride_kv[2]
    g.Hc, g.Wc = kv_compact_dims(thw, stride_kv)
    return g


class QkvCompactFn(Function):

    @staticmethod
    def forward(ctx, x, W, b, thw, stride_kv, out_dt: int, compute: int, w16, w16t):
        _need_gpu(x, W)
        x = x.contiguous()
        B, N, K = x.shape
        Cc = W.shape[0] // 3
        assert W.shape[1] == K and N == thw[0] * thw[1] * thw[2]
        g = _kv_rows_geom(B, K, thw, stride_kv)
        Nc = g.T * g.Hc * g.Wc
        xk = torch.empty(B, Nc, K, dtype=x.dtype, device=x.device)
        L.check(_lib().csts_rows_gather(C.byref(g), _p(x), _dt(x), _p(xk), _stream()), "csts_rows_gather")
        Wop = w16 if (w16 is not None and compute == BF16) else W.contiguous()
        q = torch.empty(B, N, Cc, dtype=torch_dtype(out_dt), device=x.device)
        kv = torch.empty(B, Nc, 2 * Cc, dtype=torch_dtype(out_dt), device=x.device)
        gemm(L.GEMM_NT, x, 0, K, Wop, 0, K, q, Cc, B * N, Cc, K, compute=compute, bias=(b[:Cc] if b is not None else None))
        gemm(L.GEMM_NT, xk, 0, K, Wop, Cc * K, K, kv, 2 * Cc, B * Nc, 2 * Cc, K, compute=compute,
# ... 1315 lines not shown
```

include/csts_hip.h:

```cpp
#ifndef CSTS_HIP_H
#define CSTS_HIP_H

#include <stddef.h>
#include <stdint.h>

#ifdef __cplusplus
extern "C" {
#endif

#ifndef __HIP_PLATFORM_AMD__
typedef struct ihipStream_t* hipStream_t;
#endif

enum { CSTS_F32 = 0, CSTS_BF16 = 1, CSTS_HALF = 1 };
enum { CSTS_GEMM_NT = 0, CSTS_GEMM_NN = 1, CSTS_GEMM_TN = 2 };
enum { CSTS_EPI_NONE = 0, CSTS_EPI_GELU = 1, CSTS_EPI_DGELU = 2 };
enum { CSTS_MASK_NONE = 0, CSTS_MASK_SPATIAL = 1 };

#define CSTS_ABI_VERSION 14
const char* csts_last_error(void);
int csts_abi_version(void);
int csts_half_kind(void);

typedef struct {
  int layout;
  const void* A; int a_dt; int64_t lda;
  const void* B; int b_dt; int64_t ldb;
  void* C; int c_dt; int64_t ldc;
  int64_t M, N, K;
  const float* bias;
  int epilogue;
  void* aux; int aux_dt; int64_t ldaux;
  const void* residual; int r_dt; int64_t ldr; int64_t res_row_mod;
  const float* row_scale; int64_t rows_per_scale;
  int compute;
  int split_k;
  void* workspace; size_t ws_bytes;
  float* colsum;
  int tile_rows;
  int algo;
  int res_up[6];
} csts_gemm_args;
int csts_gemm(const csts_gemm_args* args, hipStream_t stream);
size_t csts_gemm_splitk_workspace(int64_t M, int64_t N, int64_t K, int split_k);
int csts_gemm_plan(const csts_gemm_args* args, int* v2, int* tile_rows, int* nsplit);
int csts_gemm_kernel_name(const csts_gemm_args* a, char* buf, int buflen, int* nsplit);
int csts_gemm_v2_eligible(const csts_gemm_args* args);

typedef struct {
  const void* A; const void* B; float* C; float* colsum;
  int64_t lda, ldb, ldc;
  int64_t kbeg, kend;
  int M, N, m0, n0;
} csts_wgrad_item;
int csts_wgrad_grouped(const csts_wgrad_item* device_items, int nitems, int a_f32, int tile_rows, hipStream_t stream);
int csts_wgrad_grouped8(const csts_wgrad_item* device_items, int nitems, hipStream_t stream);
int csts_wgrad_grouped8_limited(const csts_wgrad_item* device_items, int nitems, int max_wgs, hipStream_t stream);
int csts_wgrad_grouped5(const csts_wgrad_item* device_items, int nitems, hipStream_t stream);

int csts_layernorm_fwd(const void* x, int x_dt, const float* gamma, const float* beta, void* y, int y_dt, float* mean,
                       float* rstd, int64_t rows, int C, float eps, hipStream_t stream);
int csts_layernorm_fwd_add(const void* x, const void* addend, void* sum_out, int x_dt, const float* gamma, const float* beta,
                           void* y, int y_dt, float* mean, float* rstd, int64_t rows, int C, float eps, hipStream_t stream);
size_t csts_layernorm_bwd_workspace(int64_t rows, int C);
int csts_layernorm_bwd(const void* dy, int dy_dt, const void* x, int x_dt, const float* gamma, const float* mean,
                       const float* rstd, void* dx, int dx_dt, const void* addend, void* dx_bf16, float* dgamma,
                       float* dbeta, void* workspace, size_t ws_bytes, int64_t rows, int C, hipStream_t stream);
int csts_layernorm_bwd_ex(const void* dy, const void* dy2, int dy_dt, const void* x, int x_dt, const float* gamma, const float* mean,
                          const float* rstd, void* dx, int dx_dt, const void* addend, void* dx_bf16,
                          const float* copy_row_scale, int64_t rows_per_scale, float* dgamma, float* dbeta,
                          void* workspace, size_t ws_bytes, int64_t rows, int C, hipStream_t stream);
int csts_layernorm_bwd2(const void* dy, int dy_dt, const void* x, int x_dt, const float* gamma0, const float* gamma1,
                        const float* mean, const float* rstd, void* dx, int dx_dt, float* dgb0, float* dgb1,
                        void* workspace, size_t ws_bytes, int64_t rows, int C, hipStream_t stream);
int csts_reduce_rows(const float* ws, float* out, int64_t nrows, int64_t ncols, float scale, hipStream_t stream);
typedef struct { const float* ws; float* out; int64_t nrows; int64_t ncols; float scale; int pad_; } csts_reduce_desc;
int csts_reduce_rows_batched(const csts_reduce_desc* device_descs, int n, int64_t max_ncols, hipStream_t stream);
int csts_reduce_rows_wide(const csts_reduce_desc* device_descs, int n, int64_t max_ncols, hipStream_t stream);

typedef struct {
  int B, C, HD;
  int Tf, Hf, Wf, Tc, Hc, Wc;
  int st, sh, sw;
  int64_t fine_batch_stride, fine_token_stride, coarse_batch_stride, coarse_token_stride;
} csts_dwconv_geom;
int csts_dwconv_strided(const csts_dwconv_geom* g, const void* fine, int fine_dt, const float* weight, void* coarse,
                        int coarse_dt, hipStream_t stream);
int csts_dwconv_transposed(const csts_dwconv_geom* g, const void* coarse, int coarse_dt, const float* weight, void* fine,
                           int fine_dt, hipStream_t stream);
size_t csts_dwconv_wgrad_workspace(const csts_dwconv_geom* g);
int csts_dwconv_wgrad(const csts_dwconv_geom* g, const void* fine, int fine_dt, const void* coarse, int coarse_dt,
                      float* dweight, void* workspace, size_t ws_bytes, hipStream_t stream);

int csts_dwconv_transposed2(const csts_dwconv_geom* g, const void* const coarse[2], int coarse_dt, const float* const weight[2],
                            void* const fine[2], int fine_dt, hipStream_t stream);
int csts_dwconv_wgrad2(const csts_dwconv_geom* g, const void* const fine[2], int fine_dt, const void* const coarse[2],
                       int coarse_dt, float* const dweight[2], void* workspace, size_t ws_bytes, hipStream_t stream);
typedef struct {
  csts_dwconv_geom geom;
  const void* fine; const void* coarse;
  void* workspace;
} csts_dwconv_wgrad_item;
#define CSTS_DWCONV_WGRAD_TABLE_ENTRY 128
size_t csts_dwconv_wgrad_grouped_workspace(const csts_dwconv_geom* g);
int csts_dwconv_wgrad_grouped_plan(const csts_dwconv_wgrad_item* items, int nitems, void* table_host, size_t table_bytes, int* nblocks);
int csts_dwconv_wgrad_grouped(const void* table_dev, int nitems, int nblocks, int dt, hipStream_t stream);

typedef struct {
  csts_dwconv_geom geom;
  int nslots;
  const void* fine[2];
  const float* weight[2]; const float* gamma[2]; const float* beta[2];
  void* conv_out[2]; void* y[2];
  float* mean[2]; float* rstd[2];
  int dt; float eps;
} csts_pool_ln_args;
int csts_pool_ln_fwd(const csts_pool_ln_args* args, hipStream_t stream);

typedef struct {
  int B, C;
  int Ti, Hi, Wi, To, Ho, Wo;
  int st, sh, sw;
} csts_pool_geom;
int csts_maxpool_fwd(const csts_pool_geom* g, const void* x, int dt, void* y, uint8_t* argmax, hipStream_t stream);
int csts_maxpool_bwd(const csts_pool_geom* g, const void* dy, int dt, const uint8_t* argmax, void* dx, hipStream_t stream);
int csts_trilinear_fwd(const csts_pool_geom* g, const void* x, int x_dt, const void* addend, int addend_dt, void* y,
                       int y_dt, hipStream_t stream);
int csts_trilinear_bwd(const csts_pool_geom* g, const void* dy, int dy_dt, void* dx, int dx_dt, hipStream_t stream);

typedef struct {
  const void* Q; const void* K; const void* V; void* O; float* LSE;
  const void* dO; float* delta; void* dQ; void* dK; void* dV;
  int dtype, B, H, Nq, Nk, head_dim;
  int64_t q_strides[3], k_strides[3], v_strides[3], o_strides[3];
  int64_t do_strides[3], dq_strides[3], dk_strides[3], dv_strides[3];
  float scale;
  int mask_mode, mask_T, mask_HW;
} csts_attn_args;
int csts_attn_fwd(const csts_attn_args* a, hipStream_t stream);
size_t csts_attn_bwd_workspace(const csts_attn_args* a);
int csts_attn_bwd(const csts_attn_args* a, void* workspace, size_t ws_bytes, hipStream_t stream);
int csts_attn_probs(const csts_attn_args* a, float* probs , hipStream_t stream);
int csts_attn_route(const csts_attn_args* a, char* buf, int buflen, int* nsplit, int* q_chunk);

typedef struct {
  int B, Cin, T, H, W;
  int kernel[3], stride[3], padding[3];
  int To, Ho, Wo;
  int Kpad;
} csts_im2col_geom;
int csts_im2col(const csts_im2col_geom* g, const void* x, int x_dt, void* col, int col_dt, hipStream_t stream);
int csts_posembed_build(const float* spatial, const float* temporal, float* pos, int T, int HW, int C, hipStream_t stream);

int csts_transpose_batched(const void* in, int in_dt, void* out, int out_dt, int64_t batch, int R, int Cc,
                           hipStream_t stream);
typedef struct { const void* src; void* dst; int R, C, r0, c0; } csts_transpose_tile;
int csts_transpose_multi(const csts_transpose_tile* device_tiles, int ntiles, hipStream_t stream);
size_t csts_colsum_workspace(int64_t batch, int64_t M, int64_t N);
int csts_colsum(const void* X, int dt, const float* row_weight, float* out, int64_t batch, int64_t M, int64_t N,
                void* workspace, size_t ws_bytes, hipStream_t stream);
int csts_axpby(const void* a, int a_dt, const void* b, int b_dt, void* out, int out_dt, int64_t n, float alpha, float beta,
               hipStream_t stream);

int csts_add2(const void* a, int a_dt, const void* b, int b_dt, float* out, void* out_bf16, int64_t n,
              hipStream_t stream);
int csts_add2_scaled_copy(const void* a, int a_dt, const void* b, int b_dt, float* out, void* out_bf16, const float* copy_scale,
                          int64_t elems_per_scale, int64_t n, hipStream_t stream);

typedef struct { int B, C, T, H, W, sh, sw, Hc, Wc; } csts_kv_rows_geom;
int csts_rows_gather(const csts_kv_rows_geom* g, const void* src, int dt, void* dst, hipStream_t stream);
int csts_rows_scatter_add(const csts_kv_rows_geom* g, const void* src, int src_dt, void* dst, int dst_dt, hipStream_t stream);

typedef struct { const void* src; void* dst; int64_t src_bs, dst_bs, src_off, dst_off; int n; int pad_; } csts_token_segment;
int csts_copy_token_segments(const csts_token_segment* segs, int nseg, int B, int C, int dt, hipStream_t stream);

int csts_scale_rows(const void* x, int x_dt, const float* row_scale, int64_t rows_per_scale, void* out, int out_dt,
                    int64_t M, int64_t N, hipStream_t stream);

int csts_dropout_fwd(const void* z, const void* residual, const float* row_scale, int64_t rows_per_scale, void* y, int dt,
                     const uint64_t* key, uint32_t site, uint32_t thr, float scale, int64_t rows, int64_t cols, hipStream_t stream);
int csts_dropout_bwd(const void* dy, int dy_dt, const float* row_scale, int64_t rows_per_scale, void* out, int out_dt,
                     const uint64_t* key, uint32_t site, uint32_t thr, float scale, int64_t rows, int64_t cols, hipStream_t stream);
int csts_dropout_mask(const uint64_t* key, uint32_t site, uint32_t thr, uint8_t* out, int64_t n, hipStream_t stream);
int csts_dropout_mask_host(uint32_t key0, uint32_t key1, uint32_t site, uint32_t thr, uint64_t first, int64_t count, uint8_t* out);

int csts_rowdot2(const void* a, int a_dt, const void* b, int b_dt, float* out, int64_t M, int C,
                 hipStream_t stream);

int csts_audio_attn_fwd(const void* qkv, int dt, float* audio_attn, float* wmap, int B, int T, int HW, int C, int H,
                        float scale, hipStream_t stream);
int csts_audio_attn_bwd(const void* qkv, int dt, const float* d_wmap, void* dqkv, int B, int T, int HW, int C, int H,
                        float scale, hipStream_t stream);

int csts_reweight_fwd(const float* x, const float* w, float* y, int64_t BT, int HW, int C, hipStream_t stream);
int csts_reweight_bwd(const float* x, const float* w, const float* dy, float* dx, float* dw, int64_t BT, int HW, int C,
                      hipStream_t stream);
int csts_token_mean_fwd(const float* x, float* out, int64_t B, int N, int C, hipStream_t stream);
int csts_token_mean_bwd(const float* dout, float* dx, int64_t B, int N, int C, hipStream_t stream);

int csts_rowdot_fwd(const void* x, int x_dt, const float* w, const float* bias, float* out, int64_t M, int C,
                    hipStream_t stream);
int csts_rowdot_dx(const float* dout, const float* w, void* dx, int dx_dt, int64_t M, int C, hipStream_t stream);
int csts_softmax_fwd(const float* x, float* p, int64_t rows, int n, float temperature, hipStream_t stream);
int csts_softmax_bwd(const float* x, const float* dp, float* dx, int64_t rows, int n, float temperature, hipStream_t stream);
int csts_kldiv_fwd(const float* p, const float* q, float* loss, float* rowloss_ws, int64_t rows, int n, float scale,
                   hipStream_t stream);
int csts_kldiv_bwd(const float* p, const float* q, const float* grad_out, float* dp, int64_t rows, int n, float scale,
                   hipStream_t stream);
int csts_rownorm_fwd(const float* a, float* a_normed, float* norms, int64_t rows, int D, float eps, hipStream_t stream);
int csts_rownorm_bwd(const float* a, const float* norms, const float* d_normed, float* da, int64_t rows, int D, float eps,
                     hipStream_t stream);
int csts_egonce_fwd(const float* sim, float* loss, float* lse_row, float* lse_col, int n, float temperature,
                    hipStream_t stream);
int csts_egonce_bwd(const float* sim, const float* lse_row, const float* lse_col, const float* grad_out, float* dsim, int n,
                    float temperature, hipStream_t stream);

typedef struct {
  void* p; void* m; void* v;
  void* w16;
  int64_t n;
  float weight_decay; int pad_;
} csts_opt_tensor;
typedef struct {
  const int32_t* chunk_tensor; const int64_t* chunk_off; int nchunks; int chunk_elems;
// ... 186 lines not shown
```

Before: 205.1 clips/s.

## Fuse attention dKV split reduction, KV-pool layernorm bwd and transposed dwconv

Adds a kv_pool_bwd kernel that consumes the attention backward's unreduced dK/dV split partials directly, folding the split reduction, the K/V layernorm backward and the transposed depthwise pooling conv into one launch. Attention backward gets a variant that skips the reduce kernel and the dK/dV outputs. The LN helpers move into a shared header so both files can use them. This removes the separate reduce pass and the round trips of the dkv and dc2 intermediates through global memory, at the cost of a more complex kernel and a host-side route query per call.

```diff
diff --git a/csts_amd/csrc/attention.hip b/csts_amd/csrc/attention.hip
--- a/csts_amd/csrc/attention.hip
+++ b/csts_amd/csrc/attention.hip
@@ -1536,16 +1536,26 @@
   return 0;
 }
 
-extern "C" int csts_attn_bwd(const csts_attn_args* a, void* workspace, size_t ws_bytes, hipStream_t stream) {
+#pragma push_macro("CSTS_FAIL")
+#undef CSTS_FAIL
+#define CSTS_FAIL(msg)                                      \
+  do {                                                      \
+    csts_set_error(std::string(who) + ": " + (msg));        \
+    return -1;                                              \
+  } while (0)
+static int attn_bwd_run(const char* who, const csts_attn_args* a, void* workspace, size_t ws_bytes, bool reduce, int* nsplit_out,
+                        hipStream_t stream) {
   ATTN_COMMON_CHECKS(a);
-  CSTS_REQUIRE(a->O && a->LSE && a->dO && a->delta && a->dQ && a->dK && a->dV, "null backward operand");
-  CSTS_REQUIRE(aligned16(a->dO) && aligned16(a->dQ) && aligned16(a->dK) && aligned16(a->dV), "alignment");
+  AttnRoute r;
+  const bool routed = attn_route(a, &r);
+  const bool need_dkv = reduce || !routed || r.nsplit == 1;
+  CSTS_REQUIRE(a->O && a->LSE && a->dO && a->delta && a->dQ && (!need_dkv || (a->dK && a->dV)), "null backward operand");
+  CSTS_REQUIRE(aligned16(a->dO) && aligned16(a->dQ) && (!need_dkv || (aligned16(a->dK) && aligned16(a->dV))), "alignment");
   CSTS_REQUIRE(strides_ok(a->do_strides, a->dtype) && strides_ok(a->dq_strides, a->dtype) &&
-                   strides_ok(a->dk_strides, a->dtype) && strides_ok(a->dv_strides, a->dtype) &&
+                   (!need_dkv || (strides_ok(a->dk_strides, a->dtype) && strides_ok(a->dv_strides, a->dtype))) &&
                    strides_ok(a->o_strides, a->dtype), "strides must keep 16-byte row alignment");
   AttnP p; fill(a, p);
-  AttnRoute r;
-  CSTS_REQUIRE(attn_route(a, &r), "no route");
+  CSTS_REQUIRE(routed, "no route");
   p.nsplit = r.nsplit; p.q_chunk = r.q_chunk;
   if (r.nsplit > 1) {
     if (workspace == nullptr || ws_bytes < r.ws_bytes) CSTS_FAIL("workspace too small [workspace != nullptr && ws_bytes >= csts_attn_bwd_workspace(a)]");
@@ -1561,11 +1571,22 @@
     CSTS_REQUIRE(LAUNCH_BY_TYPE(launch_dkv, a, r, p, grid_dkv, stream), "hipFuncSetAttribute(MaxDynamicSharedMemorySize) failed on this device");
   }
   CSTS_LAUNCH_CHECK();
-  if (r.nsplit > 1) {
+  if (r.nsplit > 1 && reduce) {
     launch_reduce(a, p, stream);
     CSTS_LAUNCH_CHECK();
   }
+  if (nsplit_out) *nsplit_out = r.nsplit;
   return 0;
+}
+#pragma pop_macro("CSTS_FAIL")
+
+extern "C" int csts_attn_bwd(const csts_attn_args* a, void* workspace, size_t ws_bytes, hipStream_t stream) {
+  return attn_bwd_run(__func__, a, workspace, ws_bytes, true, nullptr, stream);
+}
+
+extern "C" int csts_attn_bwd_splits(const csts_attn_args* a, void* workspace, size_t ws_bytes, int* nsplit, hipStream_t stream) {
+  CSTS_REQUIRE(nsplit != nullptr, "null pointer");
+  return attn_bwd_run(__func__, a, workspace, ws_bytes, false, nsplit, stream);
 }
 
 extern "C" int csts_attn_probs(const csts_attn_args* a, float* probs, hipStream_t stream) {
diff --git a/csts_amd/csrc/ln_shared.h b/csts_amd/csrc/ln_shared.h
--- /dev/null
+++ b/csts_amd/csrc/ln_shared.h
@@ -0,0 +1,257 @@
+#pragma once
+#include "common.h"
+
+#include <algorithm>
+#include <utility>
+
+namespace {
+
+constexpr int MAXV = 12;
+constexpr int LN_BWD_WAVES = 8;
+
+template <bool F32> __device__ __forceinline__ float ldt(const void* p, int64_t i) {
+  if constexpr (F32) return reinterpret_cast<const float*>(p)[i];
+  else return h16_lo((unsigned)reinterpret_cast<const unsigned short*>(p)[i]);
+}
+template <bool F32> __device__ __forceinline__ void stt(void* p, int64_t i, float v) {
+  if constexpr (F32) reinterpret_cast<float*>(p)[i] = v;
+  else reinterpret_cast<bf16*>(p)[i] = (bf16)v;
+}
+template <bool F32> __device__ __forceinline__ void ld8t(const void* p, int64_t i, float (&o)[8]) {
+  if constexpr (F32) {
+    const float4* q = reinterpret_cast<const float4*>(reinterpret_cast<const float*>(p) + i);
+    const float4 a = q[0], b = q[1];
+    o[0] = a.x; o[1] = a.y; o[2] = a.z; o[3] = a.w; o[4] = b.x; o[5] = b.y; o[6] = b.z; o[7] = b.w;
+  } else {
+    const uint4 r = *reinterpret_cast<const uint4*>(reinterpret_cast<const bf16*>(p) + i);
+    o[0] = h16_lo(r.x); o[1] = h16_hi(r.x);
+    o[2] = h16_lo(r.y); o[3] = h16_hi(r.y);
+    o[4] = h16_lo(r.z); o[5] = h16_hi(r.z);
+    o[6] = h16_lo(r.w); o[7] = h16_hi(r.w);
+  }
+}
+template <bool F32> __device__ __forceinline__ void st8t(void* p, int64_t i, const float (&o)[8]) {
+  if constexpr (F32) {
+    float4* q = reinterpret_cast<float4*>(reinterpret_cast<float*>(p) + i);
+    q[0] = make_float4(o[0], o[1], o[2], o[3]);
+    q[1] = make_float4(o[4], o[5], o[6], o[7]);
+  } else {
+    bf16x8 v;
+#pragma unroll
+    for (int j = 0; j < 8; ++j) v[j] = (bf16)o[j];
+    *reinterpret_cast<bf16x8*>(reinterpret_cast<bf16*>(p) + i) = v;
+  }
+}
+template <int W, bool F32> __device__ __forceinline__ void ldw(const void* p, int64_t i, float (&o)[W]) {
+  if constexpr (W == 8) ld8t<F32>(p, i, o);
+  else o[0] = ldt<F32>(p, i);
+}
+template <int W, bool F32> __device__ __forceinline__ void stw(void* p, int64_t i, const float (&o)[W]) {
+  if constexpr (W == 8) st8t<F32>(p, i, o);
+  else stt<F32>(p, i, o[0]);
+}
+template <int GL> __device__ __forceinline__ float group_sum(float v) {
+#pragma unroll
+  for (int o = GL / 2; o > 0; o >>= 1) v += __shfl_xor(v, o, 64);
+  return v;
+}
+
+__device__ __forceinline__ int64_t xcd_block(int64_t bid, int64_t nwg) {
+#ifdef CSTS_LN_NO_XCD_MAP
+  return bid;
+#else
+  const int64_t q = nwg >> 3, r = nwg & 7, xcd = bid & 7, slot = bid >> 3;
+  return (xcd < r ? xcd * (q + 1) : r * (q + 1) + (xcd - r) * q) + slot;
+#endif
+}
+
+template <int W, int GL, int NCH> struct Lane {
+  int sub, C;
+  int c0[W == 8 ? NCH : 1];
+  bool act[W == 8 ? NCH : 1];
+  __device__ __forceinline__ void form(int i) {
+    if constexpr (W == 8) {
+      const int c = (sub + GL * i) * 8;
+      act[i] = c < C;
+      c0[i] = min(c, C - 8);
+    }
+  }
+  __device__ __forceinline__ bool on(int i) const {
+    if constexpr (W == 8) return act[i];
+    else return sub + GL * i < C;
+  }
+  __device__ __forceinline__ int st(int i) const {
+    if constexpr (W == 8) return c0[i];
+    else return sub + GL * i;
+  }
+  __device__ __forceinline__ int at(int i) const {
+    if constexpr (W == 8) return c0[i];
+    else return min(sub + GL * i, C - 1);
+  }
+  __device__ __forceinline__ void param(const float* p, int i, float (&o)[W]) const {
+    if constexpr (W == 8) ld8t<true>(p, at(i), o);
+    else o[0] = on(i) ? p[sub + GL * i] : 0.f;
+  }
+};
+
+struct Copy16 {
+  bf16* p = nullptr;
+  const float* scale = nullptr;
+  int64_t rps = 1;
+  const void* dy2 = nullptr;
+};
+#ifndef CSTS_LN_BWD_R
+#define CSTS_LN_BWD_R 1
+#endif
+#ifndef CSTS_LN_BWD_MINW
+#define CSTS_LN_BWD_MINW 1
+#endif
+
+template <bool F32> struct DyPlain {
+  const void* dy;
+  const void* dy2;
+  int C;
+  template <int W> __device__ __forceinline__ void load(int, int64_t, int64_t row, int c, float (&o)[W]) const {
+    ldw<W, F32>(dy, row * C + c, o);
+    if (dy2) {
+      float d2[W];
+      ldw<W, F32>(dy2, row * C + c, d2);
+#pragma unroll
+      for (int j = 0; j < W; ++j) o[j] += d2[j];
+    }
+  }
+};
+
+template <int W, int GL, int NCH>
+__device__ __forceinline__ void ln_bwd_row(const Lane<W, GL, NCH>& ln, bool live, const float (&d)[NCH][W], const float (&xv)[NCH][W],
+                                           float mu, float rs, const float (&gm)[NCH][W], float invC, float (&dg)[NCH][W],
+                                           float (&db)[NCH][W], float (&o)[NCH][W]) {
+  float s1 = 0.f, s2 = 0.f;
+  float xh[NCH][W], g[NCH][W];
+#pragma unroll
+  for (int i = 0; i < NCH; ++i) {
+    const bool ok = live && ln.on(i);
+#pragma unroll
+    for (int j = 0; j < W; ++j) {
+      const float dd = ok ? d[i][j] : 0.f;
+      xh[i][j] = ok ? (xv[i][j] - mu) * rs : 0.f;
+      g[i][j] = dd * gm[i][j];
+      dg[i][j] += dd * xh[i][j];
+      db[i][j] += dd;
+      s1 += g[i][j];
+      s2 += g[i][j] * xh[i][j];
+    }
+  }
+  s1 = group_sum<GL>(s1) * invC;
+  s2 = group_sum<GL>(s2) * invC;
+#pragma unroll
+  for (int i = 0; i < NCH; ++i)
+#pragma unroll
+    for (int j = 0; j < W; ++j) o[i][j] = rs * (g[i][j] - s1 - xh[i][j] * s2);
+}
+
+template <int W, int GL, int NCH, int R, bool XF32, class DyLoad>
+__device__ __forceinline__ void ln_bwd_rows(float* red, int seg, int bx, int nbx, const DyLoad& dyl, const void* __restrict__ x,
+                                            const float* __restrict__ gamma, const float* __restrict__ mean,
+                                            const float* __restrict__ rstd, void* __restrict__ dx, const void* __restrict__ addend,
+                                            float* __restrict__ ws, int64_t rows, int C, const Copy16& dx16) {
+  const int64_t ro = (int64_t)seg * rows;
+  ws += (int64_t)seg * nbx * 2 * C;
+  const int gib = threadIdx.x / GL;
+  constexpr int GPB = 512 / GL;
+  const int64_t bid = W == 8 ? xcd_block(bx, nbx) : (int64_t)bx;
+  const int64_t grp = bid * GPB + gib, ngrp = (int64_t)nbx * GPB;
+  Lane<W, GL, NCH> ln{(int)(threadIdx.x % GL), C};
+  float gm[NCH][W], dg[NCH][W], db[NCH][W];
+#pragma unroll
+  for (int i = 0; i < NCH; ++i) {
+    ln.form(i);
+    ln.param(gamma, i, gm[i]);
+#pragma unroll
+    for (int j = 0; j < W; ++j) { dg[i][j] = 0.f; db[i][j] = 0.f; }
+  }
+  const float invC = 1.f / C;
+  for (int64_t row0 = grp * R; row0 < rows; row0 += ngrp * R) {
+    float d[R][NCH][W], xv[R][NCH][W], ad[R][NCH][W], mu[R], rs[R];
+#pragma unroll
+    for (int r = 0; r < R; ++r) {
+      const int64_t lrow = min(row0 + r, rows - 1), row = ro + lrow;
+      mu[r] = mean[row];
+      rs[r] = rstd[row];
+#pragma unroll
+      for (int i = 0; i < NCH; ++i) {
+        dyl.template load<W>(seg, lrow, row, ln.at(i), d[r][i]);
+        ldw<W, XF32>(x, row * C + ln.at(i), xv[r][i]);
+        if (addend) ldw<W, XF32>(addend, row * C + ln.at(i), ad[r][i]);
+        else {
+#pragma unroll
+          for (int j = 0; j < W; ++j) ad[r][i][j] = 0.f;
+        }
+      }
+    }
+#pragma unroll
+    for (int r = 0; r < R; ++r) {
+      const bool live = row0 + r < rows;
+      float dr[NCH][W];
+      ln_bwd_row<W, GL, NCH>(ln, live, d[r], xv[r], mu[r], rs[r], gm, invC, dg, db, dr);
+      if (live) {
+        const int64_t row = ro + row0 + r;
+#pragma unroll
+        for (int i = 0; i < NCH; ++i)
+          if (ln.on(i)) {
+            float o[W];
+#pragma unroll
+            for (int j = 0; j < W; ++j) o[j] = dr[i][j] + ad[r][i][j];
+            stw<W, XF32>(dx, row * C + ln.st(i), o);
+            if (dx16.p) {
+              if (dx16.scale) {
+                const float sc = dx16.scale[(row0 + r) / dx16.rps];
+#pragma unroll
+                for (int j = 0; j < W; ++j) o[j] *= sc;
+              }
+              stw<W, false>(dx16.p, row * C + ln.st(i), o);
+            }
+          }
+      }
+    }
+  }
+#pragma unroll
+  for (int i = 0; i < NCH; ++i)
+    if (ln.on(i)) {
+#pragma unroll
+      for (int j = 0; j < W; ++j) {
+        red[gib * 2 * C + ln.st(i) + j] = dg[i][j];
+        red[gib * 2 * C + C + ln.st(i) + j] = db[i][j];
+      }
+    }
+  __syncthreads();
+  for (int i = threadIdx.x; i < 2 * C; i += blockDim.x) {
+    float t = 0.f;
+#pragma unroll(W == 8 ? 4 : GPB)
+    for (int k = 0; k < GPB; ++k) t += red[k * 2 * C + i];
+    ws[(int64_t)bx * 2 * C + i] = t;
+  }
+}
+
+#ifndef CSTS_LN_FWD_R
+#define CSTS_LN_FWD_R 2
+#endif
+#ifndef CSTS_LN_BWD_CAP
+#define CSTS_LN_BWD_CAP 512
+#endif
+struct LnForm { int W, GL, NCH, R; };
+template <bool BWD> constexpr LnForm LN_FORMS[8] = {
+    {8, 16, 1, BWD ? CSTS_LN_BWD_R : CSTS_LN_FWD_R}, {8, 32, 1, BWD ? CSTS_LN_BWD_R : CSTS_LN_FWD_R},
+    {8, 64, 1, BWD ? CSTS_LN_BWD_R : CSTS_LN_FWD_R}, {8, 64, 2, BWD ? 1 : 2},
+    {1, 64, 2, 4}, {1, 64, 3, 4}, {1, 64, 6, 2}, {1, 64, 12, 1}};
+inline size_t ln_bwd_lds(const LnForm& f, int C) { return (size_t)(512 / f.GL) * 2 * C * sizeof(float); }
+inline int ln_form(bool bwd, int C, bool aligned) {
+  const int vec = C <= 128 ? 0 : (C <= 256 ? 1 : (C <= 512 ? 2 : 3));
+  if (aligned && C % 8 == 0 && !(bwd && ln_bwd_lds(LN_FORMS<true>[vec], C) > 65536)) return vec;
+  return 4 + (C <= 128 ? 0 : (C <= 192 ? 1 : (C <= 384 ? 2 : 3)));
+}
+inline int64_t ln_bwd_blocks(int64_t rows, int C) {
+  return std::min<int64_t>(cdiv(rows, LN_BWD_WAVES * LN_FORMS<true>[ln_form(true, C, false)].R), CSTS_LN_BWD_CAP);
+}
+
+}
diff --git a/csts_amd/csrc/norm.hip b/csts_amd/csrc/norm.hip
--- a/csts_amd/csrc/norm.hip
+++ b/csts_amd/csrc/norm.hip
@@ -1,96 +1,8 @@
-#include "common.h"
+#include "ln_shared.h"
 
 #include <utility>
 
 namespace {
-
-constexpr int MAXV = 12;
-constexpr int LN_BWD_WAVES = 8;
-
-template <bool F32> __device__ __forceinline__ float ldt(const void* p, int64_t i) {
-  if constexpr (F32) return reinterpret_cast<const float*>(p)[i];
-  else return h16_lo((unsigned)reinterpret_cast<const unsigned short*>(p)[i]);
-}
-template <bool F32> __device__ __forceinline__ void stt(void* p, int64_t i, float v) {
-  if constexpr (F32) reinterpret_cast<float*>(p)[i] = v;
-  else reinterpret_cast<bf16*>(p)[i] = (bf16)v;
-}
-template <bool F32> __device__ __forceinline__ void ld8t(const void* p, int64_t i, float (&o)[8]) {
-  if constexpr (F32) {
-    const float4* q = reinterpret_cast<const float4*>(reinterpret_cast<const float*>(p) + i);
-    const float4 a = q[0], b = q[1];
-    o[0] = a.x; o[1] = a.y; o[2] = a.z; o[3] = a.w; o[4] = b.x; o[5] = b.y; o[6] = b.z; o[7] = b.w;
-  } else {
-    const uint4 r = *reinterpret_cast<const uint4*>(reinterpret_cast<const bf16*>(p) + i);
-    o[0] = h16_lo(r.x); o[1] = h16_hi(r.x);
-    o[2] = h16_lo(r.y); o[3] = h16_hi(r.y);
-    o[4] = h16_lo(r.z); o[5] = h16_hi(r.z);
-    o[6] = h16_lo(r.w); o[7] = h16_hi(r.w);
-  }
-}
-template <bool F32> __device__ __forceinline__ void st8t(void* p, int64_t i, const float (&o)[8]) {
-  if constexpr (F32) {
-    float4* q = reinterpret_cast<float4*>(reinterpret_cast<float*>(p) + i);
-    q[0] = make_float4(o[0], o[1], o[2], o[3]);
-    q[1] = make_float4(o[4], o[5], o[6], o[7]);
-  } else {
-    bf16x8 v;
-#pragma unroll
-    for (int j = 0; j < 8; ++j) v[j] = (bf16)o[j];
-    *reinterpret_cast<bf16x8*>(reinterpret_cast<bf16*>(p) + i) = v;
-  }
-}
-template <int W, bool F32> __device__ __forceinline__ void ldw(const void* p, int64_t i, float (&o)[W]) {
-  if constexpr (W == 8) ld8t<F32>(p, i, o);
-  else o[0] = ldt<F32>(p, i);
-}
-template <int W, bool F32> __device__ __forceinline__ void stw(void* p, int64_t i, const float (&o)[W]) {
-  if constexpr (W == 8) st8t<F32>(p, i, o);
-  else stt<F32>(p, i, o[0]);
-}
-template <int GL> __device__ __forceinline__ float group_sum(float v) {
-#pragma unroll
-  for (int o = GL / 2; o > 0; o >>= 1) v += __shfl_xor(v, o, 64);
-  return v;
-}
-
-__device__ __forceinline__ int64_t xcd_block(int64_t bid, int64_t nwg) {
-#ifdef CSTS_LN_NO_XCD_MAP
-  return bid;
-#else
-  const int64_t q = nwg >> 3, r = nwg & 7, xcd = bid & 7, slot = bid >> 3;
-  return (xcd < r ? xcd * (q + 1) : r * (q + 1) + (xcd - r) * q) + slot;
-#endif
-}
-
-template <int W, int GL, int NCH> struct Lane {
-  int sub, C;
-  int c0[W == 8 ? NCH : 1];
-  bool act[W == 8 ? NCH : 1];
-  __device__ __forceinline__ void form(int i) {
-    if constexpr (W == 8) {
-      const int c = (sub + GL * i) * 8;
-      act[i] = c < C;
-      c0[i] = min(c, C - 8);
-    }
-  }
-  __device__ __forceinline__ bool on(int i) const {
-    if constexpr (W == 8) return act[i];
-    else return sub + GL * i < C;
-  }
-  __device__ __forceinline__ int st(int i) const {
-    if constexpr (W == 8) return c0[i];
-    else return sub + GL * i;
-  }
-  __device__ __forceinline__ int at(int i) const {
-    if constexpr (W == 8) return c0[i];
-    else return min(sub + GL * i, C - 1);
-  }
-  __device__ __forceinline__ void param(const float* p, int i, float (&o)[W]) const {
-    if constexpr (W == 8) ld8t<true>(p, at(i), o);
-    else o[0] = on(i) ? p[sub + GL * i] : 0.f;
-  }
-};
 
 struct FwdAdd {
   const void* addend = nullptr;
@@ -177,18 +89,6 @@
   }
 }
 
-struct Copy16 {
-  bf16* p = nullptr;
-  const float* scale = nullptr;
-  int64_t rps = 1;
-  const void* dy2 = nullptr;
-};
-#ifndef CSTS_LN_BWD_R
-#define CSTS_LN_BWD_R 1
-#endif
-#ifndef CSTS_LN_BWD_MINW
-#define CSTS_LN_BWD_MINW 1
-#endif
 template <int W, int GL, int NCH, int R, bool DYF32, bool XF32>
 __global__ __launch_bounds__(512, CSTS_LN_BWD_MINW) void ln_bwd_kernel(const void* __restrict__ dy, const void* __restrict__ x,
                                                          const float* __restrict__ gamma, const float* __restrict__ mean,
@@ -196,105 +96,9 @@
                                                          const void* __restrict__ addend, float* __restrict__ ws, int64_t rows,
                                                          int C, const float* __restrict__ gamma1, Copy16 dx16) {
   extern __shared__ __attribute__((aligned(16))) float red[];
-  const int64_t ro = (int64_t)blockIdx.y * rows;
   if (blockIdx.y == 1) gamma = gamma1;
-  ws += (int64_t)blockIdx.y * gridDim.x * 2 * C;
-  const int gib = threadIdx.x / GL;
-  constexpr int GPB = 512 / GL;
-  const int64_t bid = W == 8 ? xcd_block(blockIdx.x, gridDim.x) : (int64_t)blockIdx.x;
-  const int64_t grp = bid * GPB + gib, ngrp = (int64_t)gridDim.x * GPB;
-  Lane<W, GL, NCH> ln{(int)(threadIdx.x % GL), C};
-  float gm[NCH][W], dg[NCH][W], db[NCH][W];
-#pragma unroll
-  for (int i = 0; i < NCH; ++i) {
-    ln.form(i);
-    ln.param(gamma, i, gm[i]);
-#pragma unroll
-    for (int j = 0; j < W; ++j) { dg[i][j] = 0.f; db[i][j] = 0.f; }
-  }
-  const float invC = 1.f / C;
-  for (int64_t row0 = grp * R; row0 < rows; row0 += ngrp * R) {
-    float d[R][NCH][W], xv[R][NCH][W], ad[R][NCH][W], mu[R], rs[R];
-#pragma unroll
-    for (int r = 0; r < R; ++r) {
-      const int64_t row = ro + min(row0 + r, rows - 1);
-      mu[r] = mean[row];
-      rs[r] = rstd[row];
-#pragma unroll
-      for (int i = 0; i < NCH; ++i) {
-        ldw<W, DYF32>(dy, row * C + ln.at(i), d[r][i]);
-        if (dx16.dy2) {
-          float d2[W];
-          ldw<W, DYF32>(dx16.dy2, row * C + ln.at(i), d2);
-#pragma unroll
-          for (int j = 0; j < W; ++j) d[r][i][j] += d2[j];
-        }
-        ldw<W, XF32>(x, row * C + ln.at(i), xv[r][i]);
-        if (addend) ldw<W, XF32>(addend, row * C + ln.at(i), ad[r][i]);
-        else {
-#pragma unroll
-          for (int j = 0; j < W; ++j) ad[r][i][j] = 0.f;
-        }
-      }
-    }
-#pragma unroll
-    for (int r = 0; r < R; ++r) {
-      const bool live = row0 + r < rows;
-      float s1 = 0.f, s2 = 0.f;
-      float xh[NCH][W], g[NCH][W];
-#pragma unroll
-      for (int i = 0; i < NCH; ++i) {
-        const bool ok = live && ln.on(i);
-#pragma unroll
-        for (int j = 0; j < W; ++j) {
-          const float dd = ok ? d[r][i][j] : 0.f;
-          xh[i][j] = ok ? (xv[r][i][j] - mu[r]) * rs[r] : 0.f;
-          g[i][j] = dd * gm[i][j];
-          dg[i][j] += dd * xh[i][j];
-          db[i][j] += dd;
-          s1 += g[i][j];
-          s2 += g[i][j] * xh[i][j];
-        }
-      }
-      s1 = group_sum<GL>(s1) * invC;
-      s2 = group_sum<GL>(s2) * invC;
-      if (live) {
-        const int64_t row = ro + row0 + r;
-#pragma unroll
-        for (int i = 0; i < NCH; ++i)
-          if (ln.on(i)) {
-            float o[W];
-#pragma unroll
-            for (int j = 0; j < W; ++j) o[j] = rs[r] * (g[i][j] - s1 - xh[i][j] * s2) + ad[r][i][j];
-            stw<W, XF32>(dx, row * C + ln.st(i), o);
-            if (dx16.p) {
-              if (dx16.scale) {
-                const float sc = dx16.scale[(row0 + r) / dx16.rps];
-#pragma unroll
-                for (int j = 0; j < W; ++j) o[j] *= sc;
-              }
-              stw<W, false>(dx16.p, row * C + ln.st(i), o);
-            }
-          }
-      }
-    }
-  }
-#pragma unroll
-  for (int i = 0; i < NCH; ++i)
-    if (ln.on(i)) {
-#pragma unroll
-      for (int j = 0; j < W; ++j) {
-        red[gib * 2 * C + ln.st(i) + j] = dg[i][j];
-        red[gib * 2 * C + C + ln.st(i) + j] = db[i][j];
-      }
-    }
-  __syncthreads();
-  for (int i = threadIdx.x; i < 2 * C; i += blockDim.x) {
-    float t = 0.f;
-#pragma unroll(W == 8 ? 4 : GPB)
-    for (int k = 0; k < GPB; ++k) t += red[k * 2 * C + i];
-    ws[(int64_t)blockIdx.x * 2 * C + i] = t;
-  }
+  ln_bwd_rows<W, GL, NCH, R, XF32>(red, (int)blockIdx.y, (int)blockIdx.x, (int)gridDim.x, DyPlain<DYF32>{dy, dx16.dy2, C}, x, gamma,
+                                   mean, rstd, dx, addend, ws, rows, C, dx16);
 }
 
 template <int RL>
@@ -405,30 +209,10 @@
   return 0;
 }
 
-#ifndef CSTS_LN_FWD_R
-#define CSTS_LN_FWD_R 2
-#endif
-#ifndef CSTS_LN_BWD_CAP
-#define CSTS_LN_BWD_CAP 512
-#endif
-struct LnForm { int W, GL, NCH, R; };
-template <bool BWD> static constexpr LnForm LN_FORMS[8] = {
-    {8, 16, 1, BWD ? CSTS_LN_BWD_R : CSTS_LN_FWD_R}, {8, 32, 1, BWD ? CSTS_LN_BWD_R : CSTS_LN_FWD_R},
-    {8, 64, 1, BWD ? CSTS_LN_BWD_R : CSTS_LN_FWD_R}, {8, 64, 2, BWD ? 1 : 2},
-    {1, 64, 2, 4}, {1, 64, 3, 4}, {1, 64, 6, 2}, {1, 64, 12, 1}};
-static size_t ln_bwd_lds(const LnForm& f, int C) { return (size_t)(512 / f.GL) * 2 * C * sizeof(float); }
-static int ln_form(bool bwd, int C, bool aligned) {
-  const int vec = C <= 128 ? 0 : (C <= 256 ? 1 : (C <= 512 ? 2 : 3));
-  if (aligned && C % 8 == 0 && !(bwd && ln_bwd_lds(LN_FORMS<true>[vec], C) > 65536)) return vec;
-  return 4 + (C <= 128 ? 0 : (C <= 192 ? 1 : (C <= 384 ? 2 : 3)));
-}
 static bool all_aligned16(std::initializer_list<const void*> ptrs) {
   for (const void* q : ptrs)
     if (q != nullptr && !aligned16(q)) return false;
   return true;
-}
-static int64_t ln_bwd_blocks(int64_t rows, int C) {
-  return std::min<int64_t>(cdiv(rows, LN_BWD_WAVES * LN_FORMS<true>[ln_form(true, C, false)].R), CSTS_LN_BWD_CAP);
 }
 template <class F, int... K> static void ln_pick(int k, F&& launch, std::integer_sequence<int, K...>) {
   ((k == K ? launch(std::integral_constant<int, K>{}) : void()), ...);
diff --git a/csts_amd/csrc/stencil.hip b/csts_amd/csrc/stencil.hip
--- a/csts_amd/csrc/stencil.hip
+++ b/csts_amd/csrc/stencil.hip
@@ -1,4 +1,4 @@
-#include "common.h"
+#include "ln_shared.h"
 #include <algorithm>
 #include <cstdlib>
 #include <cstring>
@@ -354,6 +354,60 @@
   const float* w[2];
 };
 
+template <int V, bool F32> struct CoarseGlobal {
+  const void* base;
+  static constexpr int t0 = 0, h0 = 0;
+  __device__ __forceinline__ int rows(const Geom& g) const { return g.Hc; }
+  __device__ __forceinline__ Raw<V, F32> load(int i) const { return raw_load<V, F32>(base, i); }
+};
+struct CoarseLds {
+  const bf16* base;
+  int t0, h0, nh;
+  __device__ __forceinline__ int rows(const Geom&) const { return nh; }
+  __device__ __forceinline__ Raw<8, false> load(int i) const {
+    Raw<8, false> r;
+    const uint4 a = *reinterpret_cast<const uint4*>(base + i);
+    r.w[0] = a.x; r.w[1] = a.y; r.w[2] = a.z; r.w[3] = a.w;
+    return r;
+  }
+};
+
+template <int NT, int NH, int NW, bool CF32, int V, class Src>
+__device__ __forceinline__ void transposed_taps(const RowGeom& rg, const Src& src, const float* wl, int ft, int fh, int fw, int cts, int c,
+                                                int cw, float (&acc)[V]) {
+  const Geom& g = rg.g;
+  int kt[NT], ot[NT], kh[NH], oh[NH], kw[NW], ow[NW];
+  bool vt[NT], vh[NH], vw[NW];
+  axis_cand<NT>(ft, g.st, rg.lt, g.Tc, kt, ot, vt);
+  axis_cand<NH>(fh, g.sh, rg.lh, g.Hc, kh, oh, vh);
+  axis_cand<NW>(fw, g.sw, rg.lw, g.Wc, kw, ow, vw);
+#pragma unroll
+  for (int i = 0; i < NT; ++i) ot[i] = (ot[i] - src.t0) * (src.rows(g) * g.Wc * cts);
+#pragma unroll
+  for (int i = 0; i < NH; ++i) oh[i] = (oh[i] - src.h0) * (g.Wc * cts);
+#pragma unroll
+  for (int i = 0; i < NW; ++i) ow[i] = ow[i] * cts + c;
+#pragma unroll
+  for (int j = 0; j < V; ++j) acc[j] = 0.f;
+#pragma unroll
+  for (int a = 0; a < NT; ++a) {
+    Raw<V, CF32> raw[NH * NW];
+#pragma unroll
+    for (int e = 0; e < NH; ++e)
+#pragma unroll
+      for (int f = 0; f < NW; ++f) raw[e * NW + f] = src.load(ot[a] + oh[e] + ow[f]);
+#pragma unroll
+    for (int e = 0; e < NH; ++e)
+#pragma unroll
+      for (int f = 0; f < NW; ++f) {
+        const int tap = (vt[a] && vh[e] && vw[f]) ? kt[a] * 9 + kh[e] * 3 + kw[f] : 27;
+        float v[V];
+        raw_cvt<V, CF32>(raw[e * NW + f], v);
+        fmav<V>(acc, v, &wl[tap * (g.HD + WPAD) + cw]);
+      }
+  }
+}
+
 template <int NT, int NH, int NW, bool CF32, bool FF32, int V>
 __global__ __launch_bounds__(256, CSTS_DW_WAVES) void dwconv_transposed_kernel(RowGeom rg, Slots2 sl) {
   extern __shared__ __attribute__((aligned(16))) float wl[];
@@ -371,39 +425,52 @@
     const int c = (idx - bt * CQ) * V, cw = c - fdiv(c, rg.dHD) * g.HD;
     int b, ft, fh, fw;
     decompf(bt, rg.dNf, rg.dHf, rg.dWf, b, ft, fh, fw);
-    int kt[NT], ot[NT], kh[NH], oh[NH], kw[NW], ow[NW];
-    bool vt[NT], vh[NH], vw[NW];
-    axis_cand<NT>(ft, g.st, rg.lt, g.Tc, kt, ot, vt);
-    axis_cand<NH>(fh, g.sh, rg.lh, g.Hc, kh, oh, vh);
-    axis_cand<NW>(fw, g.sw, rg.lw, g.Wc, kw, ow, vw);
-#pragma unroll
-    for (int i = 0; i < NT; ++i) ot[i] *= g.Hc * g.Wc * cts;
-#pragma unroll
-    for (int i = 0; i < NH; ++i) oh[i] *= g.Wc * cts;
-#pragma unroll
-    for (int i = 0; i < NW; ++i) ow[i] = ow[i] * cts + c;
-    const void* cb = bptr<CF32>(coarse, (int64_t)b * g.c_bs);
     float acc[V];
-#pragma unroll
-    for (int j = 0; j < V; ++j) acc[j] = 0.f;
-#pragma unroll
-    for (int a = 0; a < NT; ++a) {
-      Raw<V, CF32> raw[NH * NW];
-#pragma unroll
-      for (int e = 0; e < NH; ++e)
-#pragma unroll
-        for (int f = 0; f < NW; ++f) raw[e * NW + f] = raw_load<V, CF32>(cb, ot[a] + oh[e] + ow[f]);
-#pragma unroll
-      for (int e = 0; e < NH; ++e)
-#pragma unroll
-        for (int f = 0; f < NW; ++f) {
-          const int tap = (vt[a] && vh[e] && vw[f]) ? kt[a] * 9 + kh[e] * 3 + kw[f] : 27;
-          float v[V];
-          raw_cvt<V, CF32>(raw[e * NW + f], v);
-          fmav<V>(acc, v, &wl[tap * (g.HD + WPAD) + cw]);
-        }
-    }
+    transposed_taps<NT, NH, NW, CF32, V>(rg, CoarseGlobal<V, CF32>{bptr<CF32>(coarse, (int64_t)b * g.c_bs)}, wl, ft, fh, fw, cts, c, cw, acc);
     raw_store<V, FF32>(bptr<FF32>(fine, (int64_t)b * g.f_bs), (bt - b * ntok) * fts + c, acc);
+  }
+}
+
+template <int NT, class Src>
+__device__ __forceinline__ void transposed_s22_taps(const RowGeom& rg, const Src& src, const float* wl, int ft, int mh, int mw, int cts,
+                                                    int c, int cw, float (&o00)[8], float (&o01)[8], float (&o10)[8], float (&o11)[8]) {
+  const Geom& g = rg.g;
+  int kt[NT], ot[NT];
+  bool vt[NT];
+  axis_cand<NT>(ft, g.st, rg.lt, g.Tc, kt, ot, vt);
+  const bool vh1 = mh + 1 < g.Hc, vw1 = mw + 1 < g.Wc;
+  const int oh0 = (mh - src.h0) * g.Wc * cts, oh1 = (min(mh + 1, g.Hc - 1) - src.h0) * g.Wc * cts;
+  const int ow0 = mw * cts + c, ow1 = min(mw + 1, g.Wc - 1) * cts + c;
+#pragma unroll
+  for (int j = 0; j < 8; ++j) { o00[j] = 0.f; o01[j] = 0.f; o10[j] = 0.f; o11[j] = 0.f; }
+  Raw<8, false> raw[NT][4];
+#pragma unroll
+  for (int a = 0; a < NT; ++a) {
+    const int tb = (ot[a] - src.t0) * src.rows(g) * g.Wc * cts;
+    raw[a][0] = src.load(tb + oh0 + ow0);
+    raw[a][1] = src.load(tb + oh0 + ow1);
+    raw[a][2] = src.load(tb + oh1 + ow0);
+    raw[a][3] = src.load(tb + oh1 + ow1);
+  }
+#pragma unroll
+  for (int a = 0; a < NT; ++a) {
+    float i00[8], i01[8], i10[8], i11[8];
+    raw_cvt<8, false>(raw[a][0], i00);
+    raw_cvt<8, false>(raw[a][1], i01);
+    raw_cvt<8, false>(raw[a][2], i10);
+    raw_cvt<8, false>(raw[a][3], i11);
+    const int t9 = kt[a] * 9;
+    auto wrow = [&](bool ok, int kh, int kw) { return &wl[(ok ? t9 + kh * 3 + kw : 27) * (g.HD + WPAD) + cw]; };
+    const bool v = vt[a];
+    fmav<8>(o00, i00, wrow(v, 1, 1));
+    fmav<8>(o01, i00, wrow(v, 1, 2));
+    fmav<8>(o01, i01, wrow(v && vw1, 1, 0));
+    fmav<8>(o10, i00, wrow(v, 2, 1));
+    fmav<8>(o10, i10, wrow(v && vh1, 0, 1));
+    fmav<8>(o11, i00, wrow(v, 2, 2));
+    fmav<8>(o11, i01, wrow(v && vw1, 2, 0));
+    fmav<8>(o11, i10, wrow(v && vh1, 0, 2));
+    fmav<8>(o11, i11, wrow(v && vh1 && vw1, 0, 0));
   }
 }
 
@@ -424,51 +491,152 @@
     const int c = (idx - bt * CQ) * 8, cw = c - fdiv(c, rg.dHD) * g.HD;
     int b, ft, mh, mw;
     decompf(bt, rg.dN2, rg.dH2, rg.dW2, b, ft, mh, mw);
-    int kt[NT], ot[NT];
-    bool vt[NT];
-    axis_cand<NT>(ft, g.st, rg.lt, g.Tc, kt, ot, vt);
-    const bool vh1 = mh + 1 < g.Hc, vw1 = mw + 1 < g.Wc;
-    const int oh0 = mh * g.Wc * cts, oh1 = min(mh + 1, g.Hc - 1) * g.Wc * cts;
-    const int ow0 = mw * cts + c, ow1 = min(mw + 1, g.Wc - 1) * cts + c;
-    const bf16* cb = coarse + (int64_t)b * g.c_bs;
     float o00[8], o01[8], o10[8], o11[8];
-#pragma unroll
-    for (int j = 0; j < 8; ++j) { o00[j] = 0.f; o01[j] = 0.f; o10[j] = 0.f; o11[j] = 0.f; }
-    Raw<8, false> raw[NT][4];
-#pragma unroll
-    for (int a = 0; a < NT; ++a) {
-      const int tb = ot[a] * g.Hc * g.Wc * cts;
-      raw[a][0] = raw_load<8, false>(cb, tb + oh0 + ow0);
-      raw[a][1] = raw_load<8, false>(cb, tb + oh0 + ow1);
-      raw[a][2] = raw_load<8, false>(cb, tb + oh1 + ow0);
-      raw[a][3] = raw_load<8, false>(cb, tb + oh1 + ow1);
-    }
-#pragma unroll
-    for (int a = 0; a < NT; ++a) {
-      float i00[8], i01[8], i10[8], i11[8];
-      raw_cvt<8, false>(raw[a][0], i00);
-      raw_cvt<8, false>(raw[a][1], i01);
-      raw_cvt<8, false>(raw[a][2], i10);
-      raw_cvt<8, false>(raw[a][3], i11);
-      const int t9 = kt[a] * 9;
-      auto wrow = [&](bool ok, int kh, int kw) { return &wl[(ok ? t9 + kh * 3 + kw : 27) * (g.HD + WPAD) + cw]; };
-      const bool v = vt[a];
-      fmav<8>(o00, i00, wrow(v, 1, 1));
-      fmav<8>(o01, i00, wrow(v, 1, 2));
-      fmav<8>(o01, i01, wrow(v && vw1, 1, 0));
-      fmav<8>(o10, i00, wrow(v, 2, 1));
-      fmav<8>(o10, i10, wrow(v && vh1, 0, 1));
-      fmav<8>(o11, i00, wrow(v, 2, 2));
-      fmav<8>(o11, i01, wrow(v && vw1, 2, 0));
-      fmav<8>(o11, i10, wrow(v && vh1, 0, 2));
-      fmav<8>(o11, i11, wrow(v && vh1 && vw1, 0, 0));
-    }
+    transposed_s22_taps<NT>(rg, CoarseGlobal<8, false>{coarse + (int64_t)b * g.c_bs}, wl, ft, mh, mw, cts, c, cw, o00, o01, o10, o11);
     bf16* fb = fine + (int64_t)b * g.f_bs;
     const int f00 = ((ft * g.Hf + 2 * mh) * g.Wf + 2 * mw) * fts + c;
     raw_store<8, false>(fb, f00, o00);
     raw_store<8, false>(fb, f00 + fts, o01);
     raw_store<8, false>(fb, f00 + g.Wf * fts, o10);
     raw_store<8, false>(fb, f00 + g.Wf * fts + fts, o11);
+  }
+}
+
+constexpr size_t KVP_LDS_BUDGET = 65536;
+constexpr LnForm KVP_FORM = LN_FORMS<true>[0];
+enum { KVP_S22, KVP_333, KVP_322, KVP_311 };
+
+struct DyKv {
+  const void* dkv;
+  const float* splits;
+  int nsplit;
+  int64_t per;
+  int Nk, H, HD;
+  template <int W> __device__ __forceinline__ void load(int seg, int64_t lrow, int64_t row, int c, float (&o)[W]) const {
+    static_assert(W == 8, "16-byte chunks only");
+    if (nsplit == 1) {
+      ld8t<false>(dkv, row * HD + c, o);
+      return;
+    }
+    const int l = (int)lrow, bk = l / H, head = l - bk * H, b = bk / Nk, k = bk - b * Nk;
+    const int64_t e = (((int64_t)b * H + head) * Nk + k) * HD + c;
+    float s[8] = {0.f, 0.f, 0.f, 0.f, 0.f, 0.f, 0.f, 0.f};
+    for (int sp0 = 0; sp0 < nsplit; sp0 += 4) {
+      float4 a[4], b4[4];
+#pragma unroll
+      for (int i = 0; i < 4; ++i) {
+        const float4* q = reinterpret_cast<const float4*>(splits + ((int64_t)seg * nsplit + min(sp0 + i, nsplit - 1)) * per + e);
+        a[i] = q[0]; b4[i] = q[1];
+      }
+#pragma unroll
+      for (int i = 0; i < 4; ++i)
+        if (sp0 + i < nsplit) {
+          s[0] += a[i].x; s[1] += a[i].y; s[2] += a[i].z; s[3] += a[i].w;
+          s[4] += b4[i].x; s[5] += b4[i].y; s[6] += b4[i].z; s[7] += b4[i].w;
+        }
+    }
+#pragma unroll
+    for (int j = 0; j < 8; ++j) o[j] = (float)(bf16)s[j];
+  }
+};
+
+struct KvPoolP {
+  DyKv dy;
+  int64_t rows;
+  const void* x;
+  const float* gamma[2];
+  const float* mean; const float* rstd;
+  void* dc;
+  float* lnws;
+  const float* w[2];
+  void* fine[2];
+  int nB, nbA;
+  int nhc, hrows;
+  FastDiv dCQ;
+};
+
+template <int TAP>
+__global__ __launch_bounds__(512, 4) void kv_pool_bwd_kernel(RowGeom rg, KvPoolP p) {
+  extern __shared__ __attribute__((aligned(16))) float smem[];
+  const Geom& g = rg.g;
+  const int HD = g.HD, tid = threadIdx.x;
+  if ((int)blockIdx.x >= p.nB) {
+    const int bid = (int)blockIdx.x - p.nB, seg = bid / p.nbA, bx = bid - seg * p.nbA;
+    ln_bwd_rows<KVP_FORM.W, KVP_FORM.GL, KVP_FORM.NCH, KVP_FORM.R, false>(smem, seg, bx, p.nbA, p.dy, p.x, p.gamma[seg], p.mean, p.rstd,
+                                                                          p.dc, nullptr, p.lnws, p.rows, HD, Copy16{});
+    return;
+  }
+  int bid = (int)xcd_block(blockIdx.x, p.nB);
+  const int hci = bid % p.nhc; bid /= p.nhc;
+  const int ft = bid % g.Tf; bid /= g.Tf;
+  const int head = bid % p.dy.H; bid /= p.dy.H;
+  const int b = bid % g.B, slot = bid / g.B;
+  float* wl = smem;
+  bf16* halo = reinterpret_cast<bf16*>(smem + 28 * (HD + WPAD));
+  stage_weight_rows(p.w[slot], wl, HD, 512, tid);
+  const int fh0 = hci * p.hrows, fh1 = min(fh0 + p.hrows, g.Hf);
+  const int t0 = max(ft - 1, 0), t1 = min(ft + 1, g.Tc - 1);
+  const int h0 = max(fh0 - 2, 0) / g.sh, nh = min(fh1 / g.sh, g.Hc - 1) - h0 + 1;
+  {
+    constexpr int GL = KVP_FORM.GL, GPB = 512 / GL, RH = 1;
+    Lane<8, GL, 1> ln{tid % GL, HD};
+    float gm[1][8];
+    ln.form(0);
+    ln.param(p.gamma[slot], 0, gm[0]);
+    const float invC = 1.f / HD;
+    const int nw = nh * g.Wc, nhalo = (t1 - t0 + 1) * nw;
+    for (int hr0 = (tid / GL) * RH; hr0 < nhalo; hr0 += GPB * RH) {
+      float d[RH][1][8], xv[RH][1][8], mu[RH], rs[RH];
+#pragma unroll
+      for (int r = 0; r < RH; ++r) {
+        const int hr = min(hr0 + r, nhalo - 1), pl = hr / nw, rem = hr - pl * nw, hh = rem / g.Wc, ww = rem - hh * g.Wc;
+        const int tok = ((t0 + pl) * g.Hc + h0 + hh) * g.Wc + ww;
+        const int64_t lrow = ((int64_t)b * p.dy.Nk + tok) * p.dy.H + head, row = (int64_t)slot * p.rows + lrow;
+        mu[r] = p.mean[row];
+        rs[r] = p.rstd[row];
+        p.dy.load<8>(slot, lrow, row, ln.at(0), d[r][0]);
+        ld8t<false>(p.x, row * HD + ln.at(0), xv[r][0]);
+      }
+#pragma unroll
+      for (int r = 0; r < RH; ++r) {
+        float dg[1][8], db[1][8], o[1][8];
+#pragma unroll
+        for (int j = 0; j < 8; ++j) { dg[0][j] = 0.f; db[0][j] = 0.f; }
+        ln_bwd_row<8, GL, 1>(ln, true, d[r], xv[r], mu[r], rs[r], gm, invC, dg, db, o);
+        if (hr0 + r < nhalo && ln.on(0)) {
+          float r8[8];
+#pragma unroll
+          for (int j = 0; j < 8; ++j) r8[j] = o[0][j] + 0.f;
+          st8t<false>(halo, (int64_t)(hr0 + r) * HD + ln.st(0), r8);
+        }
+      }
+    }
+  }
+  __syncthreads();
+  const CoarseLds src{halo, t0, h0, nh};
+  const int CQ = HD / 8, fts = (int)g.f_ts;
+  bf16* fb = reinterpret_cast<bf16*>(p.fine[slot]) + (int64_t)b * g.f_bs;
+  if constexpr (TAP == KVP_S22) {
+    const int W2 = g.Wf >> 1, total = ((fh1 - fh0) >> 1) * W2 * CQ;
+    for (int idx = tid; idx < total; idx += 512) {
+      const int m = fdiv(idx, p.dCQ), cw = (idx - m * CQ) * 8, mr = fdiv(m, rg.dW2), mw = m - mr * W2, mh = (fh0 >> 1) + mr;
+      float o00[8], o01[8], o10[8], o11[8];
+      transposed_s22_taps<3>(rg, src, wl, ft, mh, mw, HD, cw, cw, o00, o01, o10, o11);
+      const int f00 = ((ft * g.Hf + 2 * mh) * g.Wf + 2 * mw) * fts + head * HD + cw;
+      raw_store<8, false>(fb, f00, o00);
+      raw_store<8, false>(fb, f00 + fts, o01);
+      raw_store<8, false>(fb, f00 + g.Wf * fts, o10);
+      raw_store<8, false>(fb, f00 + g.Wf * fts + fts, o11);
+    }
+  } else {
+    constexpr int N = TAP == KVP_333 ? 3 : (TAP == KVP_322 ? 2 : 1);
+    const int total = (fh1 - fh0) * g.Wf * CQ;
+    for (int idx = tid; idx < total; idx += 512) {
+      const int tok = fdiv(idx, p.dCQ), cw = (idx - tok * CQ) * 8, fr = fdiv(tok, rg.dWf), fw = tok - fr * g.Wf, fh = fh0 + fr;
+      float acc[8];
+      transposed_taps<3, N, N, false, 8>(rg, src, wl, ft, fh, fw, HD, cw, cw, acc);
+      raw_store<8, false>(fb, ((ft * g.Hf + fh) * g.Wf + fw) * fts + head * HD + cw, acc);
+    }
   }
 }
 
@@ -1065,6 +1233,86 @@
   return transposed_launch(a, 2, coarse, coarse_dt, weight, fine, fine_dt, stream);
 }
 
+static void kv_pool_hrange(int fh0, int fh1, int s, int Hc, int* lo, int* hi) {
+  *lo = std::max(fh0 - 2, 0) / s;
+  *hi = std::min(fh1 / s, Hc - 1);
+}
+static bool kv_pool_plan(const csts_dwconv_geom* a, int dt, const float* gamma0, const float* gamma1, int* tap, size_t* lds, int* nhc,
+                         int* hrows) {
+  if (!a || dt != CSTS_BF16 || a->st != 1 || a->HD <= 0 || a->HD % 8 != 0 || a->HD > 128 || a->C <= 0 || a->C % a->HD != 0) return false;
+  if (a->Tc <= 0 || a->Hc <= 0 || a->Wc <= 0 || a->Tc != a->Tf) return false;
+  const int64_t Nk = (int64_t)a->Tc * a->Hc * a->Wc;
+  if (a->coarse_token_stride != a->C || a->coarse_batch_stride != Nk * a->C) return false;
+  if (!aligned16({gamma0, gamma1})) return false;
+  if (a->sh == 2 && a->sw == 2) *tap = (a->Hf % 2 == 0 && a->Wf % 2 == 0) ? KVP_S22 : KVP_322;
+  else if (a->sh == 1 && a->sw == 1) *tap = KVP_333;
+  else if (a->sh >= 3 && a->sw >= 3) *tap = KVP_311;
+  else return false;
+  const size_t halo = (size_t)std::min(3, a->Tc) * a->Hc * a->Wc * a->HD * sizeof(bf16);
+  if (staged_bytes(a->HD) + halo > KVP_LDS_BUDGET) return false;
+  const int nplane = 2 * a->B * (a->C / a->HD) * a->Tf;
+  int rows = (int)cdiv(a->Hf, std::max<int64_t>(1, cdiv(512, nplane)));
+  if (*tap == KVP_S22) rows += rows & 1;
+  *hrows = rows;
+  *nhc = (int)cdiv(a->Hf, rows);
+  int nh = 1;
+  for (int c = 0; c < *nhc; ++c) {
+    int lo, hi;
+    kv_pool_hrange(c * rows, std::min((c + 1) * rows, a->Hf), a->sh, a->Hc, &lo, &hi);
+    nh = std::max(nh, hi - lo + 1);
+  }
+  const size_t window = (size_t)std::min(3, a->Tc) * nh * a->Wc * a->HD * sizeof(bf16);
+  *lds = std::max(staged_bytes(a->HD) + window, ln_bwd_lds(KVP_FORM, a->HD));
+  return true;
+}
+
+extern "C" int csts_kv_pool_bwd_ok(const csts_dwconv_geom* a, int dt, const float* gamma0, const float* gamma1) {
+  int tap, nhc, hrows; size_t lds;
+  return kv_pool_plan(a, dt, gamma0, gamma1, &tap, &lds, &nhc, &hrows) && tap != KVP_S22 ? 1 : 0;
+}
+
+extern "C" int csts_kv_pool_bwd(const csts_dwconv_geom* a, int dt, const void* dkv, const float* splits, size_t splits_bytes, int nsplit,
+                                const void* x, const float* gamma0, const float* gamma1, const float* mean, const float* rstd,
+                                void* dc, const float* const weight[2], void* const fine[2], float* dgb0, float* dgb1,
+                                void* workspace, size_t ws_bytes, hipStream_t stream) {
+  CHECK_GEOM(a);
+  int tap, nhc, hrows; size_t lds;
+  CSTS_REQUIRE(kv_pool_plan(a, dt, gamma0, gamma1, &tap, &lds, &nhc, &hrows), "geometry not served");
+  CSTS_REQUIRE(weight && fine && all_set({x, gamma0, gamma1, mean, rstd, dc, workspace, weight[0], weight[1], fine[0], fine[1]}), "null pointer");
+  CSTS_REQUIRE(aligned16({x, dc, fine[0], fine[1]}), "tensors must be 16-byte aligned");
+  CSTS_REQUIRE((dgb0 == nullptr) == (dgb1 == nullptr), "dgb0/dgb1: both or neither (neither = deferred second stage)");
+  const int H = a->C / a->HD, Nk = a->Tc * a->Hc * a->Wc;
+  const int64_t rows = (int64_t)a->B * Nk * H, per = rows * a->HD;
+  CSTS_REQUIRE(nsplit >= 1, "nsplit must be >= 1");
+  if (nsplit == 1) CSTS_REQUIRE(dkv != nullptr && aligned16({dkv}), "nsplit == 1 reads dkv (16-byte aligned)");
+  else CSTS_REQUIRE(splits != nullptr && aligned16({splits}) && splits_bytes >= (size_t)2 * nsplit * per * sizeof(float),
+                    "nsplit > 1 reads 2 * nsplit slabs of B * H * Nk * HD floats");
+  const int64_t nb = ln_bwd_blocks(rows, a->HD);
+  CSTS_REQUIRE(ws_bytes >= (size_t)2 * nb * 2 * a->HD * sizeof(float), "workspace too small");
+  RowGeom rg; fill_geom(a, rg);
+  KvPoolP p{};
+  p.dy = DyKv{dkv, splits, nsplit, per, Nk, H, a->HD};
+  p.rows = rows; p.x = x; p.gamma[0] = gamma0; p.gamma[1] = gamma1; p.mean = mean; p.rstd = rstd; p.dc = dc;
+  p.lnws = reinterpret_cast<float*>(workspace);
+  for (int i = 0; i < 2; ++i) { p.w[i] = weight[i]; p.fine[i] = fine[i]; }
+  p.nhc = nhc; p.hrows = hrows;
+  p.nB = 2 * a->B * H * a->Tf * nhc; p.nbA = (int)nb;
+  p.dCQ = fast_div(a->HD / 8);
+  const dim3 grid((unsigned)(p.nB + 2 * p.nbA)), block(512);
+  switch (tap) {
+    case KVP_S22: hipLaunchKernelGGL((kv_pool_bwd_kernel<KVP_S22>), grid, block, lds, stream, rg, p); break;
+    case KVP_333: hipLaunchKernelGGL((kv_pool_bwd_kernel<KVP_333>), grid, block, lds, stream, rg, p); break;
+    case KVP_322: hipLaunchKernelGGL((kv_pool_bwd_kernel<KVP_322>), grid, block, lds, stream, rg, p); break;
+    default: hipLaunchKernelGGL((kv_pool_bwd_kernel<KVP_311>), grid, block, lds, stream, rg, p); break;
+  }
+  CSTS_LAUNCH_CHECK();
+  if (dgb0 != nullptr) {
+    csts_reduce_rows_launch(p.lnws, dgb0, nb, 2 * a->HD, 1.f, stream);
+    csts_reduce_rows_launch(p.lnws + nb * 2 * a->HD, dgb1, nb, 2 * a->HD, 1.f, stream);
+  }
+  return 0;
+}
+
 static void wgrad_plan(const csts_dwconv_geom* a, int& slab, int& nslab, int64_t& chunk, int64_t& nchunk) {
   int k = std::max(1, 192 / a->HD);
   while (k > 1 && a->C % (a->HD * k) != 0) --k;
diff --git a/csts_amd/lib.py b/csts_amd/lib.py
--- a/csts_amd/lib.py
+++ b/csts_amd/lib.py
@@ -188,6 +188,8 @@
     "csts_dwconv_wgrad_workspace": (sz, [C.POINTER(DwconvGeom)]),
     "csts_dwconv_wgrad": (_I, [C.POINTER(DwconvGeom), vp, _I, vp, _I, vp, vp, sz, vp]),
     "csts_dwconv_transposed2": (_I, [C.POINTER(DwconvGeom), vp * 2, _I, vp * 2, vp * 2, _I, vp]),
+    "csts_kv_pool_bwd_ok": (_I, [C.POINTER(DwconvGeom), _I, vp, vp]),
+    "csts_kv_pool_bwd": (_I, [C.POINTER(DwconvGeom), _I, vp, vp, sz, _I, vp, vp, vp, vp, vp, vp, vp * 2, vp * 2, vp, vp, vp, sz, vp]),
     "csts_dwconv_wgrad2": (_I, [C.POINTER(DwconvGeom), vp * 2, _I, vp * 2, _I, vp * 2, vp, sz, vp]),
     "csts_dwconv_wgrad_grouped_workspace": (sz, [C.POINTER(DwconvGeom)]),
     "csts_dwconv_wgrad_grouped_plan": (_I, [C.POINTER(DwconvWgradItem), _I, vp, sz, C.POINTER(C.c_int)]),
@@ -200,6 +202,7 @@
     "csts_attn_fwd": (_I, [C.POINTER(AttnArgs), vp]),
     "csts_attn_bwd_workspace": (sz, [C.POINTER(AttnArgs)]),
     "csts_attn_bwd": (_I, [C.POINTER(AttnArgs), vp, sz, vp]),
+    "csts_attn_bwd_splits": (_I, [C.POINTER(AttnArgs), vp, sz, C.POINTER(_I), vp]),
     "csts_attn_probs": (_I, [C.POINTER(AttnArgs), vp, vp]),
     "csts_attn_route": (_I, [C.POINTER(AttnArgs), C.c_char_p, _I, C.POINTER(_I), C.POINTER(_I)]),
     "csts_im2col": (_I, [C.POINTER(Im2colGeom), vp, _I, vp, _I, vp]),
diff --git a/csts_amd/ops.py b/csts_amd/ops.py
--- a/csts_amd/ops.py
+++ b/csts_amd/ops.py
@@ -1083,6 +1083,16 @@
     return a
 
 
+def _kv_pool_bwd_ok(lib, g, dt, gk, gv) -> bool:
+    return bool(lib.csts_kv_pool_bwd_ok(C.byref(g), dt, _p(gk), _p(gv)))
+
+
+def _attn_nsplit(lib, a) -> int:
+    buf, nsplit, q_chunk = C.create_string_buffer(256), C.c_int(0), C.c_int(0)
+    L.check(lib.csts_attn_route(C.byref(a), buf, len(buf), C.byref(nsplit), C.byref(q_chunk)), "csts_attn_route")
+    return nsplit.value
+
+
 class AttnInnerFn(Function):
 
     @staticmethod
@@ -1205,15 +1215,25 @@
             return dqkv, slot * Cc, (N * QW, QW, HD)
 
         tq = grad_target(0, Nq)
-        if "kv" in saved:
+        dims, mask = (B, H, Nq, Nk, HD), (mask_mode, mask_T, mask_HW)
+        kv_fused = "kv" in saved and _kv_pool_bwd_ok(lib, saved["kv"][3], _dt(qkv), gk, gv)
+        nsplit = _attn_nsplit(lib, _attn_args(_dt(qkv), dims, mask, qd, kd, vd)) if kv_fused else 1
+        dkv = None
+        if "kv" in saved and nsplit == 1:
             dkv = torch.empty(2, B, Nk, Cc, dtype=qkv.dtype, device=dev)
             tk, tv = (dkv[0], 0, (Nk * Cc, Cc, HD)), (dkv[1], 0, (Nk * Cc, Cc, HD))
+        elif "kv" in saved:
+            tk = tv = None
         else:
             tk, tv = grad_target(1, Nk), grad_target(2, Nk)
-        a = _attn_args(_dt(qkv), (B, H, Nq, Nk, HD), (mask_mode, mask_T, mask_HW), qd, kd, vd, o=o, lse=lse, do=do, delta=delta,
-                       tq=tq, tk=tk, tv=tv)
+        a = _attn_args(_dt(qkv), dims, mask, qd, kd, vd, o=o, lse=lse, do=do, delta=delta, tq=tq, tk=tk, tv=tv)
         ws = _ws(lib.csts_attn_bwd_workspace(C.byref(a)), dev)
-        L.check(lib.csts_attn_bwd(C.byref(a), _p(ws), ws.numel(), s), "csts_attn_bwd")
+        if kv_fused:
+            got = C.c_int(0)
+            L.check(lib.csts_attn_bwd_splits(C.byref(a), _p(ws), ws.numel(), C.byref(got), s), "csts_attn_bwd_splits")
+            assert got.value == nsplit, (got.value, nsplit)
+        else:
+            L.check(lib.csts_attn_bwd(C.byref(a), _p(ws), ws.numel(), s), "csts_attn_bwd")
 
         grads = {}
 
@@ -1261,17 +1281,22 @@
             nbytes = lib.csts_layernorm_bwd_workspace(rows, HD)
             lws = _ws(2 * nbytes, dev)
             defer = _can_defer(P[3], P[4], P[5], P[6], P[7], P[8])
-            L.check(lib.csts_layernorm_bwd2(_p(dkv), _dt(dkv), _p(c2), _dt(c2), _p(gk), _p(gv), _p(mean2), _p(rstd2), _p(dc2),
-                                            _dt(dc2), None if defer else _p(dgb[0]), None if defer else _p(dgb[1]), _p(lws),
-                                            lws.numel(), rows, HD, s), "csts_layernorm_bwd2")
+            vp2 = C.c_void_p * 2
+            dgb_p = (None, None) if defer else (_p(dgb[0]), _p(dgb[1]))
+            fine_p = vp2(_p(kv_dfine, kv_off[0]), _p(kv_dfine, kv_off[1]))
+            if kv_fused:
+                L.check(lib.csts_kv_pool_bwd(C.byref(g), _dt(c2), _p(dkv), _p(ws) if nsplit > 1 else None, ws.numel(), nsplit, _p(c2),
+                                             _p(gk), _p(gv), _p(mean2), _p(rstd2), _p(dc2), vp2(_p(wk), _p(wv)), fine_p, dgb_p[0],
+                                             dgb_p[1], _p(lws), lws.numel(), s), "csts_kv_pool_bwd")
+            else:
+                L.check(lib.csts_layernorm_bwd2(_p(dkv), _dt(dkv), _p(c2), _dt(c2), _p(gk), _p(gv), _p(mean2), _p(rstd2), _p(dc2),
+                                                _dt(dc2), dgb_p[0], dgb_p[1], _p(lws), lws.numel(), rows, HD, s), "csts_layernorm_bwd2")
+                L.check(lib.csts_dwconv_transposed2(C.byref(g), vp2(_p(dc2[0]), _p(dc2[1])), _dt(dc2), vp2(_p(wk), _p(wv)), fine_p,
+                                                    _dt(kv_dfine), s), "csts_dwconv_transposed2")
             if defer:
                 nrow = nbytes // (2 * HD * 4)
                 _defer(lws[:nbytes], dgb[0], nrow, 2 * HD)
                 _defer(lws[nbytes:], dgb[1], nrow, 2 * HD)
-            vp2 = C.c_void_p * 2
-            L.check(lib.csts_dwconv_transposed2(C.byref(g), vp2(_p(dc2[0]), _p(dc2[1])), _dt(dc2), vp2(_p(wk), _p(wv)),
-                                                vp2(_p(kv_dfine, kv_off[0]), _p(kv_dfine, kv_off[1])), _dt(kv_dfine), s),
-                    "csts_dwconv_transposed2")
             grouped = defer and _stencil_group_now()
             wsz = (lib.csts_dwconv_wgrad_grouped_workspace if grouped else lib.csts_dwconv_wgrad_workspace)(C.byref(g))
             wws = _ws(2 * wsz, dev)
diff --git a/include/csts_hip.h b/include/csts_hip.h
--- a/include/csts_hip.h
+++ b/include/csts_hip.h
@@ -96,6 +96,11 @@
                             void* const fine[2], int fine_dt, hipStream_t stream);
 int csts_dwconv_wgrad2(const csts_dwconv_geom* g, const void* const fine[2], int fine_dt, const void* const coarse[2],
                        int coarse_dt, float* const dweight[2], void* workspace, size_t ws_bytes, hipStream_t stream);
+int csts_kv_pool_bwd_ok(const csts_dwconv_geom* g, int dt, const float* gamma0, const float* gamma1);
+int csts_kv_pool_bwd(const csts_dwconv_geom* g, int dt, const void* dkv, const float* splits, size_t splits_bytes, int nsplit,
+                     const void* x, const float* gamma0, const float* gamma1, const float* mean, const float* rstd, void* dc,
+                     const float* const weight[2], void* const fine[2], float* dgb0, float* dgb1, void* workspace,
+                     size_t ws_bytes, hipStream_t stream);
 typedef struct {
   csts_dwconv_geom geom;
   const void* fine; const void* coarse;
@@ -140,6 +145,7 @@
 int csts_attn_fwd(const csts_attn_args* a, hipStream_t stream);
 size_t csts_attn_bwd_workspace(const csts_attn_args* a);
 int csts_attn_bwd(const csts_attn_args* a, void* workspace, size_t ws_bytes, hipStream_t stream);
+int csts_attn_bwd_splits(const csts_attn_args* a, void* workspace, size_t ws_bytes, int* nsplit, hipStream_t stream);
 int csts_attn_probs(const csts_attn_args* a, float* probs , hipStream_t stream);
 int csts_attn_route(const csts_attn_args* a, char* buf, int buflen, int* nsplit, int* q_chunk);
 
```

After: 204.8 clips/s. No clear change (-0.2%).
